# alessiodevoto/peekvit

Measured on AMD Instinct MI355X. Metric: images/sec ViT-B/16 fwd @ batch 2048, 224x224, higher is better.
Workload: dtype f16; 1 GPU; vit_b_16 forward, batch 2048/GPU, 224x224; global_batch=2048, parallelism=replicas x1 (batch-sharded, no collective), precision_mode=auto, streams=1, operands=IEEE fp16 operands, fp32 accumulate (same MFMA rate as bf16), range-guarded, range_guard_fallbacks=0

## Files before the change

### peekvit_amd/_build.py

```python
from __future__ import annotations

import glob
import os
import subprocess
import sys

HERE = os.path.dirname(os.path.abspath(__file__))
CSRC = os.path.join(HERE, "csrc")
LIB = os.path.join(HERE, "libpeekvit_hip.so")
LIB_F16 = os.path.join(HERE, "libpeekvit_hip_f16.so")
HIPCC = os.environ.get("HIPCC", "/opt/rocm/bin/hipcc")
FLAGS = ["--offload-arch=gfx950", "-O3", "-std=c++17", "-fPIC", "-Wno-unused-result"]
HEADERS = ("peekvit_hip.h", "peekvit_hip_moe.h", "peekvit_hip_ee.h", "peekvit_hip_sparse.h", "peekvit_hip_pct.h",
           "peekvit_hip_pct_train.h", "peekvit_hip_attn_stream.h", "peekvit_hip_pct_block.h", "peekvit_hip_rank_train.h", "peekvit_hip_rank_infer.h",
           "peekvit_hip_avit_train.h", "peekvit_hip_sparse_train.h", "peekvit_hip_avit_pack_train.h", "peekvit_hip_dropout.h", "peekvit_hip_sparse_long.h",
           "peekvit_hip_sparse_long_train.h", "peekvit_hip_avit_long.h")
FILE_FLAGS = {"pv_attention.hip": ["-mllvm", "-amdgpu-mfma-vgpr-form=1"], "pv_rowops.hip": ["-fno-slp-vectorize"],
              "pv_attention_stream.hip": ["-mllvm", "-amdgpu-mfma-vgpr-form=1"],
              "pv_ee.hip": ["-fno-slp-vectorize"],
              "pv_sparse.hip": ["-fno-slp-vectorize"],
              "pv_sparse_long.hip": ["-fno-slp-vectorize"],
              "pv_pct.hip": ["-fno-slp-vectorize"],
              "pv_pct_train.hip": ["-fno-slp-vectorize"],
              "pv_rank_train.hip": ["-fno-slp-vectorize"],
              "pv_avit_train.hip": ["-fno-slp-vectorize"],
              "pv_avit_pack_train.hip": ["-fno-slp-vectorize"],
              "pv_avit_long.hip": ["-fno-slp-vectorize"],
              "pv_dropout.hip": ["-fno-slp-vectorize"],
              "pv_sparse_train.hip": ["-fno-slp-vectorize", "-mllvm", "-amdgpu-mfma-vgpr-form=1"],
              "pv_sparse_long_train.hip": ["-fno-slp-vectorize"]}


def sources():
    return sorted(glob.glob(os.path.join(CSRC, "*.hip")))


def _stale() -> bool:
    if not os.path.exists(LIB) or not os.path.exists(LIB_F16):
        return True
    t = min(os.path.getmtime(LIB), os.path.getmtime(LIB_F16))
    deps = sources() + glob.glob(os.path.join(CSRC, "*.h")) + [os.path.join(os.path.dirname(HERE), "include", h) for h in HEADERS] + [os.path.abspath(__file__)]
    return any(os.path.getmtime(d) > t for d in deps)


def build(force: bool = False, verbose: bool = False) -> str:
    if not force and not _stale():
        return LIB
    procs = []
    variants = [("build", [], LIB), ("build_f16", ["-DPV_OPERAND_F16"], LIB_F16)]
    objs = {lib: [] for _, _, lib in variants}
    for sub, defs, lib in variants:
        objdir = os.path.join(HERE, sub)
        os.makedirs(objdir, exist_ok=True)
        for src in sources():
            obj = os.path.join(objdir, os.path.basename(src)[:-4] + ".o")
            objs[lib].append(obj)
            cmd = [HIPCC, *FLAGS, *FILE_FLAGS.get(os.path.basename(src), []), *defs, "-c", src, "-o", obj]
            if verbose:
                print(" ".join(cmd))
            procs.append((src, subprocess.Popen(cmd, stdout=subprocess.PIPE, stderr=subprocess.STDOUT)))
    for src, p in procs:
        out, _ = p.communicate()
        if p.returncode != 0:
            raise RuntimeError(f"hipcc failed on {src}:\n{out.decode(errors='replace')}")
    for _, _, lib in variants:
        cmd = [HIPCC, "--offload-arch=gfx950", "-shared", "-fPIC", "-o", lib, *objs[lib]]
        r = subprocess.run(cmd, stdout=subprocess.PIPE, stderr=subprocess.STDOUT)
        if r.returncode != 0:
            raise RuntimeError(f"link failed:\n{r.stdout.decode(errors='replace')}")
    return LIB


def build_variant(tag: str, defs, force: bool = False) -> str:
    lib = os.path.join(HERE, f"libpeekvit_hip_{tag}.so")
    deps = sources() + glob.glob(os.path.join(CSRC, "*.h")) + [os.path.join(os.path.dirname(HERE), "include", h) for h in HEADERS]
    if not force and os.path.exists(lib) and all(os.path.getmtime(d) <= os.path.getmtime(lib) for d in deps):
        return lib
    objdir = os.path.join(HERE, "build_" + tag)
    os.makedirs(objdir, exist_ok=True)
    procs, objs = [], []
    for src in sources():
        obj = os.path.join(objdir, os.path.basename(src)[:-4] + ".o")
        objs.append(obj)
        procs.append((src, subprocess.Popen([HIPCC, *FLAGS, *FILE_FLAGS.get(os.path.basename(src), []), *defs, "-c", src, "-o", obj],
                                            stdout=subprocess.PIPE, stderr=subprocess.STDOUT)))
    for src, p in procs:
        out, _ = p.communicate()
        if p.returncode != 0:
            raise RuntimeError(f"hipcc failed on {src}:\n{out.decode(errors='replace')}")
    r = subprocess.run([HIPCC, "--offload-arch=gfx950", "-shared", "-fPIC", "-o", lib, *objs], stdout=subprocess.PIPE, stderr=subprocess.STDOUT)
    if r.returncode != 0:
        raise RuntimeError(f"link failed:\n{r.stdout.decode(errors='replace')}")
    return lib


if __name__ == "__main__":
    print(build(force="--force" in sys.argv, verbose=True))
```

### peekvit_amd/_lib.py

```python
from __future__ import annotations

import ctypes as C
import os
import threading

import torch

from ._build import LIB

_i64, _f32, _p, _i32 = C.c_int64, C.c_float, C.c_void_p, C.c_int32

PV_EPI_BIAS_BF16, PV_EPI_BIAS_GELU_BF16, PV_EPI_BIAS_RES_F32, PV_EPI_BIAS_POS_F32 = 0, 1, 2, 3
PV_EPI_BIAS_F32, PV_EPI_BIAS_GELU_SPLIT_BF16 = 4, 5
PV_EPI_BIAS_GELU_PAIR_BF16, PV_EPI_GELU_GRAD_BF16 = 6, 7
PV_WS_TRANSPOSE_COLSUM, PV_WS_COLSUM, PV_WS_LAYERNORM_BWD, PV_WS_GEMM_COLSUM_PARTIAL, PV_WS_GEMM_SPLITK = 1, 2, 3, 4, 5


class GemmArgs(C.Structure):
    _fields_ = [("struct_size", C.c_uint64), ("A", _p), ("W", _p), ("bias", _p), ("out", _p), ("res", _p), ("row_scale", _p), ("pos", _p),
                ("M", _i64), ("N", _i64), ("K", _i64), ("lda", _i64), ("ldw", _i64), ("ldo", _i64), ("ldr", _i64),
                ("rows_per_img_in", _i64), ("rows_per_img_out", _i64), ("row_off", _i64), ("qcols", _i64),
                ("qscale", _f32), ("epilogue", _i32),
                ("ln_gamma", _p), ("ln_beta", _p), ("ln_row_scale", _p), ("ln_out", _p), ("ln_eps", _f32),
                ("ksplit", _i32), ("colsum_partial", _p),
# ... 86 lines not shown
    "pv_layernorm_f32_bf16": (C.c_int, [_p, _i64, _p, _p, _p, _p, _i64, _i64, _i64, _f32, _p]),
    "pv_mean_pool_f32": (C.c_int, [_p, _p, _i64, _i64, _i64, _p]),
    "pv_pct_head_f32": (C.c_int, [_p, _p, _p, _p, _p, _p, _p, _p, _i64, _i64, _i64, _i64, _p]),
}

SIGNATURES_PCT_TRAIN = {
    "pv_arpe_knn": (C.c_int, [_p, _p, _i64, _i64, _i64, _p]),
    "pv_arpe_pair_moments": (C.c_int, [_p, _p, _p, _p, _i64, _i64, _i64, _p]),
    "pv_arpe_pair_max": (C.c_int, [_p, _p, _p, _p, _p, _p, _p, _p, _i64, _i64, _i64, _p]),
    "pv_arpe_pair_bwd": (C.c_int, [_p, _p, _p, _p, _p, _p, _p, _i64, _i64, _p]),
}

SIGNATURES_ATTN_STREAM = {
    "pv_attention_stream_lse_bf16": (C.c_int, [_p, _p, _p, _i64, _i64, _i64, _i64, _p, _p]),
    "pv_attention_stream_bwd_bf16": (C.c_int, [_p, _p, _p, _p, _p, _p, _i64, _i64, _i64, _i64, _f32, _p]),
}

SIGNATURES_PCT_BLOCK = {
    "pv_layernorm_bwd_sum": (C.c_int, [_p, _p, _p, _p, _p, _p, _p, _p, _i64, _i64, _i64, _f32, C.c_int, _p]),
    "pv_attention_stream_bwd16_bf16": (C.c_int, [_p, _p, _p, _p, _p, _p, _p, _i64, _i64, _i64, _i64, _f32, _p]),
}

SIGNATURES_RANK_TRAIN = {
    "pv_rank_pack_f32": (C.c_int, [_p, _p, _p, _i64, _i64, _i64, _i64, _p]),
    "pv_rank_expand_f32": (C.c_int, [_p, _p, _i64, _i64, _i64, _i64, _p]),
    "pv_rank_reduce_f32": (C.c_int, [_p, _p, _i64, _i64, _i64, _i64, _p]),
    "pv_rank_unpack_grad_f32": (C.c_int, [_p, _p, _p, _i64, _i64, _i64, _i64, _p]),
    "pv_layernorm_f32_bf16_masked": (C.c_int, [_p, _p, _p, _p, _p, _p, _i64, _i64, _f32, _p]),
    "pv_layernorm_bwd_sum_masked": (C.c_int, [_p, _p, _p, _p, _p, _p, _p, _p, _p, _i64, _i64, _i64, _f32, C.c_int, _p]),
    "pv_attention_stream_lse_w_bf16": (C.c_int, [_p, _p, _p, _i64, _i64, _i64, _i64, _f32, _p, _p]),
    "pv_attention_stream_bwd16_w_bf16": (C.c_int, [_p, _p, _p, _p, _p, _p, _p, _i64, _i64, _i64, _i64, _f32, _f32, _p]),
}

SIGNATURES_RANK_INFER = {
    "pv_rank_order_gap": (C.c_int, [_p, _p, _p, _i64, _i64, _i64, _p]),
    "pv_layernorm_gather_f32_bf16": (C.c_int, [_p, _p, _p, _p, _p, _p, _i64, _i64, _i64, _i64, _f32, _p]),
}

SIGNATURES_AVIT_TRAIN = {
    "pv_avit_act_fwd": (C.c_int, [_p] * 16 + [_i64, _i64, _i64, _i64, _f32, _f32, _f32, C.c_int, _p]),
    "pv_avit_act_bwd": (C.c_int, [_p] * 9 + [_i64, _i64, _i64, _i64, _f32, C.c_int, _p]),
}

SIGNATURES_SPARSE_TRAIN = {
    "pv_attention_varlen_w_lse_bf16": (C.c_int, [_p, _p, _p, _p, _p, _i64, _i64, _i64, _i64, _p, _p]),
    "pv_attention_varlen_w_bwd16_bf16": (C.c_int, [_p, _p, _p, _p, _p, _p, _p, _p, _p, _i64, _i64, _i64, _i64, _f32, _p]),
    "pv_residual_pack_step_train": (C.c_int, [_p, _p, _p, _p, _i64, _i64, _i64, _p, _p, _p, _p, _f32, _f32, _p,
                                              _p, _p, _p, _p, _p, _p, _p, _p, _p, _p, _p, _f32, _p, _p, _p, _p]),
    "pv_residual_pack_step_bwd": (C.c_int, [_p] * 11 + [_i64, _i64, _i64, _p, _p, _f32, _p, _p, _p, _p, _p, _p]),
}

SIGNATURES_AVIT_PACK_TRAIN = {
    "pv_avit_pack_step_train": (C.c_int, [_p] * 4 + [_i64] * 4 + [_p] * 12 + [_i64, _p, _f32, _f32, _f32, C.c_int] + [_p] * 11),
    "pv_avit_pack_step_bwd": (C.c_int, [_p] * 16 + [_i64] * 6 + [_f32, C.c_int, _p]),
}

_u64 = C.c_uint64
SIGNATURES_DROPOUT = {
    "pv_dropout_keep_u8": (C.c_int, [_p, _u64, _u64, _i64, _i64, _f32, _p]),
    "pv_dropout_f32": (C.c_int, [_p, _p, _u64, _u64, _i64, _i64, _f32, _p]),
    "pv_dropout_residual": (C.c_int, [_p, _p, _p, _u64, _u64, _i64, _i64, _f32, _p]),
    "pv_dropout_bwd16": (C.c_int, [_p, _p, _u64, _u64, _i64, _i64, _f32, _p]),
    "pv_attention_stream_lse_drop_bf16": (C.c_int, [_p, _p, _p, _i64, _i64, _i64, _i64, _f32, _u64, _u64, _p, _p]),
    "pv_attention_stream_bwd16_drop_bf16": (C.c_int, [_p, _p, _p, _p, _p, _p, _p, _i64, _i64, _i64, _i64, _f32, _f32, _u64, _u64, _p]),
}

SIGNATURES_SPARSE_LONG = {
    "pv_attention_varlen_w_stream_bf16": SIGNATURES_SPARSE["pv_attention_varlen_w_bf16"],
    "pv_residual_pack_step_long": SIGNATURES_SPARSE["pv_residual_pack_step"],
}

SIGNATURES_SPARSE_LONG_TRAIN = {
    "pv_attention_varlen_w_stream_lse_bf16": SIGNATURES_SPARSE_TRAIN["pv_attention_varlen_w_lse_bf16"],
    "pv_attention_varlen_w_stream_bwd16_bf16": SIGNATURES_SPARSE_TRAIN["pv_attention_varlen_w_bwd16_bf16"],
    "pv_residual_pack_step_long_train": SIGNATURES_SPARSE_TRAIN["pv_residual_pack_step_train"],
    "pv_residual_pack_step_long_bwd": SIGNATURES_SPARSE_TRAIN["pv_residual_pack_step_bwd"],
}

SIGNATURES_AVIT_LONG = {
    "pv_avit_pack_step_long": SIGNATURES_AVIT_PACK_TRAIN["pv_avit_pack_step_train"],
    "pv_avit_pack_step_long_bwd": SIGNATURES_AVIT_PACK_TRAIN["pv_avit_pack_step_bwd"],
}

ABI_VERSION = 10
_lock = threading.Lock()
_libs: dict = {}

_OPERAND_DEFAULT = "bf16"
_tls = threading.local()
LIB_F16 = os.path.join(os.path.dirname(os.path.abspath(__file__)), "libpeekvit_hip_f16.so")


def current_operand() -> str:
    return getattr(_tls, "operand", _OPERAND_DEFAULT)


def set_operand(op: str) -> str:
    old = current_operand()
    _tls.operand = op
    return old


def __getattr__(name):
    if name == "OPERAND":
        return current_operand()
    raise AttributeError(f"module {__name__!r} has no attribute {name!r}")


def operand_dtype():
    import torch as _t
    return _t.float16 if current_operand() == "f16" else _t.bfloat16


class PeekvitHipError(RuntimeError):
    pass


def lib_path(operand: str = "bf16") -> str:
    return LIB_F16 if operand == "f16" else LIB


def load(operand=None):
    op = current_operand() if operand is None else operand
    lib = _libs.get(op)
    if lib is not None:
        return lib
    with _lock:
        lib = _libs.get(op)
        if lib is not None:
            return lib
        path = lib_path(op)
        if not os.path.exists(path):
            raise PeekvitHipError(
                f"{path} not found: the MI355X kernels are not built. Run `python -m peekvit_amd._build` "
                "(or __graft_entry__.build()); there is no fallback path.")
        lib = C.CDLL(path)
        for name, (res, args) in {**SIGNATURES, **SIGNATURES_MOE, **SIGNATURES_EE, **SIGNATURES_SPARSE, **SIGNATURES_PCT,
                                   **SIGNATURES_PCT_TRAIN, **SIGNATURES_ATTN_STREAM, **SIGNATURES_PCT_BLOCK, **SIGNATURES_RANK_TRAIN,
                                   **SIGNATURES_RANK_INFER, **SIGNATURES_AVIT_TRAIN, **SIGNATURES_SPARSE_TRAIN, **SIGNATURES_AVIT_PACK_TRAIN,
                                   **SIGNATURES_DROPOUT, **SIGNATURES_SPARSE_LONG, **SIGNATURES_SPARSE_LONG_TRAIN,
                                   **SIGNATURES_AVIT_LONG}.items():
            fn = getattr(lib, name)
            fn.restype, fn.argtypes = res, args
        if lib.pv_version() != ABI_VERSION:
            raise PeekvitHipError(f"{path} has ABI v{lib.pv_version()}, this package binds v{ABI_VERSION}: rebuild (python -m peekvit_amd._build)")
        if lib.pv_gemm_args_size() != C.sizeof(GemmArgs):
            raise PeekvitHipError(f"{path}: pv_gemm_args is {lib.pv_gemm_args_size()} bytes in the library, {C.sizeof(GemmArgs)} in this binding")
        if lib.pv_operand_type() != (1 if op == "f16" else 0):
            raise PeekvitHipError(f"{path} was built for a different operand type")
        _libs[op] = lib
    return lib


def check(code: int, what: str = "") -> None:
    if code != 0:
        msg = load().pv_error_string(code).decode()
        raise PeekvitHipError(f"{what}: {msg} (code {code})" if what else f"{msg} (code {code})")
```

### peekvit_amd/csrc/pv_gemm.hip

```cpp
#include "pv_rows.h"
#include "../../include/peekvit_hip_moe.h"
#include "pv_gelu_table.h"
#include <type_traits>
#include <cstdlib>

typedef __attribute__((ext_vector_type(8))) short s16x8;

#ifndef PV_STORE_NT
#define PV_STORE_NT 3
#endif
#define PV_STORE16(ptr, val) do { if (PV_STORE_NT & 1) __builtin_nontemporal_store((val), (ptr)); else *(ptr) = (val); } while (0)
#define PV_STORE32(ptr, val) do { if (PV_STORE_NT & 2) __builtin_nontemporal_store((val), (ptr)); else *(ptr) = (val); } while (0)
#ifndef PV_PF_MODE
#define PV_PF_MODE 2
#endif
#ifndef PV_EPI_PIPE
#define PV_EPI_PIPE 1
#endif

__device__ __forceinline__ float pv_fma_s(float a, float b, float c) {
    float r;
    asm("v_fma_f32 %0, %1, %2, %3" : "=v"(r) : "v"(a), "v"(b), "v"(c));
    return r;
}
__device__ __forceinline__ float pv_mul_s(float a, float b) {
    float r;
    asm("v_mul_f32 %0, %1, %2" : "=v"(r) : "v"(a), "v"(b));
    return r;
}
__device__ __forceinline__ float pv_gelu_poly(float x, const f32x4 c) {
    const pv_f32x2_t c02 = {c[0], c[1]}, c13 = {c[2], c[3]}, xx = {x, x};
    const pv_f32x2_t r = __builtin_elementwise_fma(c13, xx, c02);
    return pv_fma_s(x, pv_mul_s(x, r[1]), r[0]);
}
__device__ __forceinline__ void pv_gelu_bits2(float x0, float x1, uint32_t& b0, uint32_t& b1) {
    const pv_f32x2_t xs = {x0, x1}, sc = {PV_GELU_CUB_SCALE, PV_GELU_CUB_SCALE}, mg = {PV_GELU_CUB_MAGIC, PV_GELU_CUB_MAGIC};
    const pv_f32x2_t t = __builtin_elementwise_fma(xs, sc, mg);
    typedef __attribute__((ext_vector_type(2))) int pv_i32x2_t;
    const pv_i32x2_t ti = __builtin_bit_cast(pv_i32x2_t, t);
    const int lo = 0x4B400000, hi = 0x4B400000 + PV_GELU_CUB_N - 1;
    b0 = (uint32_t)min(max(ti[0], lo), hi);
    b1 = (uint32_t)min(max(ti[1], lo), hi);
}
#ifndef PV_GELU_GLOBAL_MODE
#define PV_GELU_GLOBAL_MODE 1
#endif
__device__ __forceinline__ float pv_gelu_poly_g(float x, f32x4 c) {
#if PV_GELU_GLOBAL_MODE == 0
    return pv_gelu_poly(x, c);
#elif PV_GELU_GLOBAL_MODE == 2
    asm volatile("s_nop 3" : "+v"(c));
    return pv_gelu_poly(x, c);
#elif PV_GELU_GLOBAL_MODE == 3
    pv_f32x2_t r;
    const pv_f32x2_t c02 = {c[0], c[1]}, c13 = {c[2], c[3]}, xx = {x, x};
    asm volatile("v_pk_fma_f32 %0, %1, %2, %3" : "=&v"(r) : "v"(c13), "v"(xx), "v"(c02));
    return pv_fma_s(x, pv_mul_s(x, r[1]), r[0]);
#elif PV_GELU_GLOBAL_MODE == 4
    const pv_f32x2_t c02 = {c[0], c[1]}, c13 = {c[2], c[3]}, xx = {x, x};
    const pv_f32x2_t r = __builtin_elementwise_fma(c13, xx, c02);
    return fmaf(x, x * r[1], r[0]);
#elif PV_GELU_GLOBAL_MODE == 6
    pv_f32x2_t r;
    const pv_f32x2_t c02 = {c[0], c[1]}, c13 = {c[2], c[3]}, xx = {x, 0.0f};
    asm volatile("v_pk_fma_f32 %0, %1, %2, %3 op_sel_hi:[1,0,1]" : "=&v"(r) : "v"(c13), "v"(xx), "v"(c02));
    return pv_fma_s(x, pv_mul_s(x, r[1]), r[0]);
#elif PV_GELU_GLOBAL_MODE == 9
    pv_f32x2_t r;
    const pv_f32x2_t c02 = {c[0], c[1]}, c13 = {c[2], c[3]}, xx = {0.0f, x};
    asm volatile("v_pk_fma_f32 %0, %1, %2, %3 op_sel:[0,1,0]" : "=&v"(r) : "v"(c13), "v"(xx), "v"(c02));
    return pv_fma_s(x, pv_mul_s(x, r[1]), r[0]);
#elif PV_GELU_GLOBAL_MODE == 7
    pv_f32x2_t c02 = {c[0], c[1]};
    const pv_f32x2_t c13 = {c[2], c[3]}, xx = {x, x};
    asm volatile("v_pk_fma_f32 %0, %1, %2, %0" : "+v"(c02) : "v"(c13), "v"(xx));
    return pv_fma_s(x, pv_mul_s(x, c02[1]), c02[0]);
#elif PV_GELU_GLOBAL_MODE == 8
    pv_f32x2_t c13 = {c[2], c[3]};
    const pv_f32x2_t c02 = {c[0], c[1]}, xx = {x, x};
    asm volatile("v_pk_fma_f32 %0, %0, %1, %2" : "+v"(c13) : "v"(xx), "v"(c02));
    return pv_fma_s(x, pv_mul_s(x, c13[1]), c13[0]);
#elif PV_GELU_GLOBAL_MODE == 5
    const float r0 = pv_fma_s(c[2], x, c[0]), r1 = pv_fma_s(c[3], x, c[1]);
    return pv_fma_s(x, pv_mul_s(x, r1), r0);
#else
    const float r0 = fmaf(c[2], x, c[0]), r1 = fmaf(c[3], x, c[1]);
    return pv_fma_s(x, pv_mul_s(x, r1), r0);
#endif
}
__device__ __forceinline__ void pv_gelu_lut2(float& x0, float& x1, const f32x4* tab) {
    uint32_t b0, b1;
    pv_gelu_bits2(x0, x1, b0, b1);
    const f32x4 c0 = tab[(b0 - 0x4B400000u) * PV_GELU_CUB_REP], c1 = tab[(b1 - 0x4B400000u) * PV_GELU_CUB_REP];
    x0 = pv_gelu_poly_g(x0, c0); x1 = pv_gelu_poly_g(x1, c1);
}
__device__ __forceinline__ void pv_gelu_lut2(float& x0, float& x1, const __attribute__((address_space(3))) f32x4* tab) {
    uint32_t b0, b1;
    pv_gelu_bits2(x0, x1, b0, b1);
    const uint32_t base = (uint32_t)(uintptr_t)tab - 0x40000000u;
    const f32x4 c0 = *(const __attribute__((address_space(3))) f32x4*)(uintptr_t)((b0 << 8) + base);
    const f32x4 c1 = *(const __attribute__((address_space(3))) f32x4*)(uintptr_t)((b1 << 8) + base);
    x0 = pv_gelu_poly(x0, c0); x1 = pv_gelu_poly(x1, c1);
}

__device__ __forceinline__ float pv_gelu_dpoly(float x, const f32x4 c) {
    const float t = pv_fma_s(pv_mul_s(c[3], 3.0f), x, pv_add_s(c[1], c[1]));
    return pv_fma_s(x, t, c[2]);
}
__device__ __forceinline__ void pv_gelu_dlut2(float& x0, float& x1, const f32x4* tab) {
    uint32_t b0, b1;
    pv_gelu_bits2(x0, x1, b0, b1);
    const f32x4 c0 = tab[(b0 - 0x4B400000u) * PV_GELU_CUB_REP], c1 = tab[(b1 - 0x4B400000u) * PV_GELU_CUB_REP];
    x0 = pv_gelu_dpoly(x0, c0); x1 = pv_gelu_dpoly(x1, c1);
}
__device__ __forceinline__ void pv_gelu_dlut2(float& x0, float& x1, const __attribute__((address_space(3))) f32x4* tab) {
    uint32_t b0, b1;
    pv_gelu_bits2(x0, x1, b0, b1);
    const uint32_t base = (uint32_t)(uintptr_t)tab - 0x40000000u;
    const f32x4 c0 = *(const __attribute__((address_space(3))) f32x4*)(uintptr_t)((b0 << 8) + base);
    const f32x4 c1 = *(const __attribute__((address_space(3))) f32x4*)(uintptr_t)((b1 << 8) + base);
    x0 = pv_gelu_dpoly(x0, c0); x1 = pv_gelu_dpoly(x1, c1);
}

struct GemmDev {
    const uint16_t* A;
    const uint16_t* W;
    const float* bias;
    void* out;
    const float* res;
    const float* row_scale;
    const float* pos;
    int M, N, K;
    int64_t lda, ldw, ldo, ldr;
    int rpi, rpo, row_off, qcols;
    float qscale;
    int tiles_m, tiles_n;
    int fr_full, fr_half;
    int fr_big;
    int gm;
    int gc;
    uint32_t* range_flag;
    float* rowsq_out;
    int res_scaled;
    int k_last;
    float* colsum_partial;
    uint16_t* x16_out;
    float* rowstat_out;
    const float* fold_stat;
    const float* fold_c1;
    const float* fold_c2;
    int ksplit;
    int k_slice;
    int64_t split_stride;
    const float* ln_gamma;
    const float* ln_beta;
    const float* ln_row_scale;
    uint16_t* ln_out;
    float ln_eps;
    const int* row_map;
    int map_rows;
#ifdef PV_STAMPS
    unsigned long long* dbg;
#endif
};

#ifdef PV_STAMPS
static unsigned long long* g_pv_dbg = nullptr;
extern "C" void pv_debug_set_stamp_buffer(void* p) { g_pv_dbg = (unsigned long long*)p; }
#define PV_STAMP(i)                                                                                  \
    do {                                                                                             \
        __builtin_amdgcn_sched_barrier(0);                                                           \
        unsigned long long t_;                                                                       \
        asm volatile("s_memtime %0\n\ts_waitcnt lgkmcnt(0)" : "=s"(t_)::"memory");                    \
        __builtin_amdgcn_sched_barrier(0);                                                           \
        if (threadIdx.x == 0 && p.dbg) p.dbg[pv_stamp_slot * 16 + (i)] = t_;                         \
    } while (0)
#else
#define PV_STAMP(i)
#endif

template <int AUX = 0>
__device__ __forceinline__ void pv_glds16(const void* gsrc, void* lds_wave_base) {
    __builtin_amdgcn_global_load_lds((const __attribute__((address_space(1))) void*)gsrc,
                                     (__attribute__((address_space(3))) void*)lds_wave_base, 16, 0, AUX);
}
#ifndef PV_GEMM_A_AUX
#define PV_GEMM_A_AUX 0
#endif
#ifndef PV_GEMM_W_AUX
#define PV_GEMM_W_AUX 0
#endif

__device__ __forceinline__ int pv_xcd_remap(int bid, int nwg) {
    const int q = nwg >> 3, r = nwg & 7, xcd = bid & 7, i = bid >> 3;
    return (xcd < r ? xcd * (q + 1) : r * (q + 1) + (xcd - r) * q) + i;
}

template <int EPI>
__device__ __forceinline__ f32x4 pv_epilogue_fetch(const GemmDev& p, int m, int n) {
    m = m < p.M ? m : p.M - 1;
    n = n + 4 <= p.N ? n : p.N - 4;
    if (EPI == PV_EPI_BIAS_RES_F32) {
        return *reinterpret_cast<const f32x4*>(p.res + (int64_t)m * p.ldr + n);
    } else if (EPI == PV_EPI_GELU_GRAD_BF16) {
        const u32x2 w = *reinterpret_cast<const u32x2*>(reinterpret_cast<const uint16_t*>(p.res) + (int64_t)m * p.ldr + n);
        return (f32x4){pv_unpack_lo(w[0]), pv_unpack_hi(w[0]), pv_unpack_lo(w[1]), pv_unpack_hi(w[1])};
    } else if (EPI == PV_EPI_BIAS_POS_F32) {
        const int img = m / p.rpi, pi = m - img * p.rpi;
        return *reinterpret_cast<const f32x4*>(p.pos + (int64_t)(p.row_off + pi) * p.N + n);
    }
    return (f32x4){0.f, 0.f, 0.f, 0.f};
}

template <int EPI, bool GUARD = true>
__device__ __forceinline__ void pv_epilogue_store(const GemmDev& p, int m, int n, f32x4 acc, f32x4 r, float row_scale, float& vmax) {
    if (GUARD && (m >= p.M || n >= p.N)) return;
    const float v0 = acc[0], v1 = acc[1], v2 = acc[2], v3 = acc[3];
    if (EPI == PV_EPI_BIAS_BF16) {
        const float s = n < p.qcols ? p.qscale : 1.0f;
        u32x2 o = {pv_pack_bf16x2_tracked(v0 * s, v1 * s, vmax), pv_pack_bf16x2_tracked(v2 * s, v3 * s, vmax)};
        *reinterpret_cast<u32x2*>(reinterpret_cast<uint16_t*>(p.out) + (int64_t)m * p.ldo + n) = o;
    } else if (EPI == PV_EPI_BIAS_GELU_BF16) {
        const f32x4* tab = reinterpret_cast<const f32x4*>(pv_gelu_cub) + (threadIdx.x & 15);
        float y0 = v0, y1 = v1, y2 = v2, y3 = v3;
        pv_gelu_lut2(y0, y1, tab); pv_gelu_lut2(y2, y3, tab);
        u32x2 o = {pv_pack_bf16x2_tracked(y0, y1, vmax), pv_pack_bf16x2_tracked(y2, y3, vmax)};
        *reinterpret_cast<u32x2*>(reinterpret_cast<uint16_t*>(p.out) + (int64_t)m * p.ldo + n) = o;
    } else if (EPI == PV_EPI_BIAS_RES_F32) {
        const float s = row_scale, t = p.res_scaled ? row_scale : 1.0f;
        float4 o = make_float4(fmaf(s, v0, t * r[0]), fmaf(s, v1, t * r[1]), fmaf(s, v2, t * r[2]), fmaf(s, v3, t * r[3]));
        *reinterpret_cast<float4*>(reinterpret_cast<float*>(p.out) + (int64_t)m * p.ldo + n) = o;
    } else if (EPI == PV_EPI_BIAS_F32) {
        const float s = n < p.qcols ? p.qscale : 1.0f;
        *reinterpret_cast<float4*>(reinterpret_cast<float*>(p.out) + (int64_t)m * p.ldo + n) = make_float4(v0 * s, v1 * s, v2 * s, v3 * s);
    } else if (EPI == PV_EPI_BIAS_GELU_SPLIT_BF16) {
        const f32x4* tab = reinterpret_cast<const f32x4*>(pv_gelu_cub) + (threadIdx.x & 15);
        float y0 = v0, y1 = v1, y2 = v2, y3 = v3;
        pv_gelu_lut2(y0, y1, tab); pv_gelu_lut2(y2, y3, tab);
        const PvHiLo a = pv_split2(y0, y1), b = pv_split2(y2, y3);
        uint16_t* o = reinterpret_cast<uint16_t*>(p.out) + (int64_t)m * p.ldo + n;
        *reinterpret_cast<u32x2*>(o) = (u32x2){a.hi, b.hi};
        *reinterpret_cast<u32x2*>(o + p.N) = (u32x2){a.lo, b.lo};
        *reinterpret_cast<u32x2*>(o + 2 * p.N) = (u32x2){a.hi, b.hi};
    } else if (EPI == PV_EPI_BIAS_GELU_PAIR_BF16) {
        const f32x4* tab = reinterpret_cast<const f32x4*>(pv_gelu_cub) + (threadIdx.x & 15);
        uint16_t* o = reinterpret_cast<uint16_t*>(p.out) + (int64_t)m * p.ldo + n;
        float y0 = v0, y1 = v1, y2 = v2, y3 = v3, d0 = v0, d1 = v1, d2 = v2, d3 = v3;
// ... 214 lines not shown
            bf16x8 xf[4], wf[4];
#pragma unroll
            for (int t = 0; t < 4; ++t) {
                xf[t] = *reinterpret_cast<const bf16x8*>(la + a_off + t * 2048 + fx);
                wf[t] = *reinterpret_cast<const bf16x8*>(lw + w_off + t * 2048 + fx);
            }
#pragma unroll
            for (int nt = 0; nt < 4; ++nt)
#pragma unroll
                for (int mt = 0; mt < 4; ++mt)
                    acc[nt][mt] = PV_MFMA_16x16x32(wf[nt], xf[mt], acc[nt][mt], 0, 0, 0);
        }
        if (kt + 1 < nk) put(cur ^ 1);
        asm volatile("s_waitcnt vmcnt(0)" ::: "memory");
        __syncthreads();
    }

    const int em = m0 + wm * 64 + (lane & 15);
    float dummy = 0.f;
    f32x4 rr[4][4];
#pragma unroll
    for (int mt = 0; mt < 4; ++mt)
#pragma unroll
        for (int nt = 0; nt < 4; ++nt) rr[mt][nt] = pv_epilogue_fetch<EPI>(p, em + mt * 16, en + nt * 16);
#pragma unroll
    for (int mt = 0; mt < 4; ++mt)
#pragma unroll
        for (int nt = 0; nt < 4; ++nt) asm volatile("" : "+v"(rr[mt][nt]));
    __builtin_amdgcn_sched_barrier(0);
    if (m0 + G1_BM <= p.M && n0 + G1_BN <= p.N) {
#pragma unroll
        for (int mt = 0; mt < 4; ++mt)
#pragma unroll
            for (int nt = 0; nt < 4; ++nt) pv_epilogue_store<EPI, false>(p, em + mt * 16, en + nt * 16, acc[nt][mt], rr[mt][nt], 1.0f, dummy);
    } else {
#pragma unroll
        for (int mt = 0; mt < 4; ++mt)
#pragma unroll
            for (int nt = 0; nt < 4; ++nt) pv_epilogue_store<EPI, true>(p, em + mt * 16, en + nt * 16, acc[nt][mt], rr[mt][nt], 1.0f, dummy);
    }
    pv_range_commit(vmax, p.range_flag);
}

extern "C" int pv_patch_embed_f32(const float* img, const uint16_t* W, const float* bias, const float* pos, float* tokens, int64_t B, int64_t C, int64_t R,
                                  int64_t P, int64_t D, int64_t S, int64_t row_off, uint32_t* range_flag, void* stream) {
    if (!img || !W || !pos || !tokens || B <= 0 || C <= 0 || R <= 0 || P <= 0 || D <= 0 || S <= 0 || row_off < 0) return PV_ERR_INVALID_ARG;
    if (R % P || P % 8 || (C * P * P) % G1_BK || D % 4 || R % 4 || ((uintptr_t)img & 15) || ((uintptr_t)W & 15) || ((uintptr_t)tokens & 15) || ((uintptr_t)pos & 15) ||
        (bias && ((uintptr_t)bias & 15)))
        return PV_ERR_UNSUPPORTED;
    const int64_t Wp = R / P, Np = Wp * Wp, M = B * Np;
    if (row_off + Np > S || M > 0x7fffffff || B * S > 0x7fffffff) return PV_ERR_INVALID_ARG;
    GemmDev p = {};
    p.W = W; p.bias = bias; p.out = tokens; p.pos = pos;
    p.M = (int)M; p.N = (int)D; p.K = (int)(C * P * P);
    p.ldw = p.K; p.ldo = D;
    p.rpi = (int)Np; p.rpo = (int)S; p.row_off = (int)row_off;
    p.qscale = 1.0f;
    p.tiles_m = (int)((M + G1_BM - 1) / G1_BM); p.tiles_n = (int)((D + G1_BN - 1) / G1_BN);
    p.range_flag = range_flag;
    const PatchGeom gm = {img, (int)C, (int)R, (int)P, (int)Wp, (int)Np};
    static PvPerDevice attr_set;
    const int lds = 2 * 2 * G1_TILE_BYTES;
    if (attr_set.first_use()) (void)hipFuncSetAttribute(reinterpret_cast<const void*>(pv_patch_embed_kernel), hipFuncAttributeMaxDynamicSharedMemorySize, lds);
    PV_LAUNCH(pv_patch_embed_kernel, dim3((unsigned)(p.tiles_m * p.tiles_n)), dim3(256), lds, (hipStream_t)stream, p, gm);
    return pv_check_launch();
}

template <int EPI>
static int pv_launch_gemm128(const GemmDev& p, hipStream_t stream) {
    static PvPerDevice attr_set;
    const int lds = 2 * 2 * G1_TILE_BYTES;
    if (attr_set.first_use()) {
        (void)hipFuncSetAttribute(reinterpret_cast<const void*>(pv_gemm128_kernel<EPI>), hipFuncAttributeMaxDynamicSharedMemorySize, lds);
    }
    PV_LAUNCH(pv_gemm128_kernel<EPI>, dim3((unsigned)(p.tiles_m * p.tiles_n * (p.ksplit > 1 ? p.ksplit : 1))), dim3(256), lds, stream, p);
    return pv_check_launch();
}

constexpr int G2_BM = 256, G2_BN = 256, G2_BK = 64;
constexpr int G2_HALF = 128 * G2_BK * 2;
constexpr int G2_BUF = 4 * G2_HALF;
constexpr int G2_LDS = 2 * G2_BUF;

template <int EPI, bool PF = false, bool FULL = false, bool PERM = false>
__device__ __forceinline__ void pv_gemm256_tile(const GemmDev& p, char* smem, const int m0, const int n0, const bool first = true,
                                                const bool has_next = false, const int nm0 = 0, const int nn0 = 0, const int wid_pf = 0, const int slot_pf = 0) {
    int tid_ = threadIdx.x;
    if (PF) {
        int l_;
        asm volatile("v_mbcnt_lo_u32_b32 %0, -1, 0\n\tv_mbcnt_hi_u32_b32 %0, -1, %0" : "=v"(l_));
        tid_ = wid_pf * 64 + l_;
    }
    int tid = tid_, lane = tid & 63;
    const int wid = PF ? wid_pf : __builtin_amdgcn_readfirstlane(tid >> 6);
    const int wr = wid >> 2, wc = wid & 3;
#ifdef PV_STAMPS
    const size_t pv_stamp_slot = PF ? (size_t)slot_pf : (size_t)blockIdx.x;
#endif
    constexpr int PFM = PV_PF_MODE;
    constexpr int PF_BIAS_BASE = G2_LDS + ((EPI == PV_EPI_BIAS_GELU_BF16 || EPI == PV_EPI_BIAS_GELU_SPLIT_BF16 || EPI == PV_EPI_BIAS_GELU_PAIR_BF16) ? PV_GELU_CUB_N * PV_GELU_CUB_REP * 16 : 0) + 4096;
    PV_STAMP(14);
#ifdef PV_STAMPS
    if (threadIdx.x == 0 && p.dbg) { unsigned long long rt_; asm volatile("s_memrealtime %0\n\ts_waitcnt lgkmcnt(0)" : "=s"(rt_)::"memory"); p.dbg[pv_stamp_slot * 16 + 13] = rt_; }
#endif

    const int srow = wid * 8 + (lane >> 3);
    const int schunk = (lane & 7) ^ ((lane >> 3) & 7);
    const char* const a_blk = reinterpret_cast<const char*>(p.A + (int64_t)m0 * p.lda);
    const char* const w_blk = reinterpret_cast<const char*>(p.W + (int64_t)n0 * p.ldw);
    uint32_t oa[2][2], ow[2][2];
#pragma unroll
    for (int h = 0; h < 2; ++h)
#pragma unroll
        for (int j = 0; j < 2; ++j) {
            int ra = h * 128 + j * 64 + srow; ra = (FULL || m0 + ra < p.M) ? ra : p.M - 1 - m0;
            const int q = j * 64 + srow;
            int rw = h * 128 + (q & ~31) + (((q & 15) >> 2) << 3) + (((q >> 4) & 1) << 2) + (q & 3);
            rw = (FULL || n0 + rw < p.N) ? rw : p.N - 1 - n0;
            oa[h][j] = (uint32_t)(ra * (int)p.lda + schunk * 8) * 2u;
            ow[h][j] = (uint32_t)(rw * (int)p.ldw + schunk * 8) * 2u;
        }
    char* const lds_piece = smem + wid * 1024;
    auto stage_a = [&](int buf, int h, int kt) {
        const char* src = a_blk + kt * (G2_BK * 2);
        pv_glds16<PV_GEMM_A_AUX>(src + oa[h][0], lds_piece + buf * G2_BUF + h * G2_HALF);
        pv_glds16<PV_GEMM_A_AUX>(src + oa[h][1], lds_piece + buf * G2_BUF + h * G2_HALF + 8192);
    };
    auto stage_b = [&](int buf, int h, int kt) {
        const char* src = w_blk + kt * (G2_BK * 2);
        pv_glds16<PV_GEMM_W_AUX>(src + ow[h][0], lds_piece + buf * G2_BUF + (2 + h) * G2_HALF);
        pv_glds16<PV_GEMM_W_AUX>(src + ow[h][1], lds_piece + buf * G2_BUF + (2 + h) * G2_HALF + 8192);
    };
    auto stage_next_piece = [&](int tm0, int tn0, int pc) __attribute__((always_inline)) {
        if (pc == 8) {
            if (p.bias && wid < 4) {
                const int c_ = tn0 + wid * 64 + lane < p.N ? tn0 + wid * 64 + lane : p.N - 1;
                __builtin_amdgcn_global_load_lds((const __attribute__((address_space(1))) void*)(p.bias + c_),
                                                 (__attribute__((address_space(3))) void*)(smem + PF_BIAS_BASE + wid * 256), 4, 0, 0);
            }
            return;
        }
        const int h = (pc >> 1) & 1, jj = pc & 1;
        const int sr = wid * 8 + (lane >> 3), sc = (lane & 7) ^ ((lane >> 3) & 7);
        if (pc < 4) {
            const char* const na = reinterpret_cast<const char*>(p.A + (int64_t)tm0 * p.lda);
            int ra = h * 128 + jj * 64 + sr; ra = tm0 + ra < p.M ? ra : p.M - 1 - tm0;
            pv_glds16<PV_GEMM_A_AUX>(na + (uint32_t)(ra * (int)p.lda + sc * 8) * 2u, lds_piece + h * G2_HALF + jj * 8192);
        } else {
            const char* const nw = reinterpret_cast<const char*>(p.W + (int64_t)tn0 * p.ldw);
            const int q = jj * 64 + sr;
            int rw = h * 128 + (q & ~31) + (((q & 15) >> 2) << 3) + (((q >> 4) & 1) << 2) + (q & 3);
            rw = tn0 + rw < p.N ? rw : p.N - 1 - tn0;
            pv_glds16<PV_GEMM_W_AUX>(nw + (uint32_t)(rw * (int)p.ldw + sc * 8) * 2u, lds_piece + (2 + h) * G2_HALF + jj * 8192);
        }
    };

    typedef __attribute__((address_space(3))) const char lds_cc;
    const int frow = (lane & 15) * 128;
    const int fx0 = ((lane >> 4) ^ (lane & 7)) << 4;
    lds_cc* const lds0 = (lds_cc*)smem;
    lds_cc* a_rd[2][2];
    lds_cc* b_rd[2][2];
#pragma unroll
    for (int b = 0; b < 2; ++b)
#pragma unroll
        for (int ks = 0; ks < 2; ++ks) {
            a_rd[b][ks] = lds0 + b * G2_BUF + wr * G2_HALF + frow + (fx0 ^ (ks << 6));
// ... 335 lines not shown
            if (pass == 1) {
                asm volatile("s_waitcnt lgkmcnt(0)" ::: "memory");
                __builtin_amdgcn_s_barrier();
            }
#pragma unroll
            for (int mt = 0; mt < 8; ++mt) {
                const int row = wr * 128 + mt * 16 + i16;
                float f_mean = 0.f, f_rstd = 1.f;
                if ((EPI == PV_EPI_BIAS_BF16 || EPI == PV_EPI_BIAS_GELU_BF16) && p.fold_stat) { f_mean = f_mean8[mt]; f_rstd = f_rstd8[mt]; }
#pragma unroll
                for (int u = 0; u < 2; ++u) {
                    f32x4 lo = acc[2 * u][mt], hi = acc[2 * u + 1][mt];
                    if ((EPI == PV_EPI_BIAS_BF16 || EPI == PV_EPI_BIAS_GELU_BF16) && p.fold_stat) {
#pragma unroll
                        for (int e = 0; e < 4; ++e) {
                            lo[e] = fmaf(f_rstd, fmaf(-f_mean, fc1[u][0][e], lo[e]), fc2[u][0][e]);
                            hi[e] = fmaf(f_rstd, fmaf(-f_mean, fc1[u][1][e], hi[e]), fc2[u][1][e]);
                        }
                    }
                    const float qs = (EPI == PV_EPI_BIAS_BF16 && en0 + u * 32 < p.qcols) ? p.qscale : 1.0f;
                    u32x4 pk;
                    if (PAIR) {
                        {
                            const __attribute__((address_space(3))) f32x4* tab = (const __attribute__((address_space(3))) f32x4*)(cimg + G2_LDS) + i16;
#pragma unroll
                            for (int e = 0; e < 4; e += 2) {
                                float t0 = lo[e], t1 = lo[e + 1], t2 = hi[e], t3 = hi[e + 1];
                                if (pass == 1) { pv_gelu_lut2(t0, t1, tab); pv_gelu_lut2(t2, t3, tab); }
                                else { pv_gelu_dlut2(t0, t1, tab); pv_gelu_dlut2(t2, t3, tab); }
                                lo[e] = t0; lo[e + 1] = t1; hi[e] = t2; hi[e + 1] = t3;
                            }
                        }
                        pk = (u32x4){pv_pack_bf16x2_tracked(lo[0], lo[1], vmax), pv_pack_bf16x2_tracked(lo[2], lo[3], vmax),
                                     pv_pack_bf16x2_tracked(hi[0], hi[1], vmax), pv_pack_bf16x2_tracked(hi[2], hi[3], vmax)};
                    } else if (EPI == PV_EPI_BIAS_GELU_BF16 || EPI == PV_EPI_BIAS_GELU_SPLIT_BF16) {
                        if (pass == 0) {
                            const __attribute__((address_space(3))) f32x4* tab = (const __attribute__((address_space(3))) f32x4*)(cimg + G2_LDS) + i16;
#pragma unroll
                            for (int e = 0; e < 4; e += 2) {
                                float t0 = lo[e], t1 = lo[e + 1], t2 = hi[e], t3 = hi[e + 1];
                                pv_gelu_lut2(t0, t1, tab); pv_gelu_lut2(t2, t3, tab);
                                lo[e] = t0; lo[e + 1] = t1; hi[e] = t2; hi[e + 1] = t3;
                            }
                            if (SPLIT) { acc[2 * u][mt] = lo; acc[2 * u + 1][mt] = hi; }
                        }
                        if (SPLIT) {
                            const PvHiLo s0 = pv_split2(lo[0], lo[1]), s1 = pv_split2(lo[2], lo[3]), s2 = pv_split2(hi[0], hi[1]), s3 = pv_split2(hi[2], hi[3]);
                            pk = pass == 0 ? (u32x4){s0.hi, s1.hi, s2.hi, s3.hi} : (u32x4){s0.lo, s1.lo, s2.lo, s3.lo};
                        } else {
                            pk = (u32x4){pv_pack_bf16x2_tracked(lo[0], lo[1], vmax), pv_pack_bf16x2_tracked(lo[2], lo[3], vmax),
                                         pv_pack_bf16x2_tracked(hi[0], hi[1], vmax), pv_pack_bf16x2_tracked(hi[2], hi[3], vmax)};
                        }
                    } else {
                        pk = (u32x4){pv_pack_bf16x2_tracked(lo[0] * qs, lo[1] * qs, vmax), pv_pack_bf16x2_tracked(lo[2] * qs, lo[3] * qs, vmax),
                                     pv_pack_bf16x2_tracked(hi[0] * qs, hi[1] * qs, vmax), pv_pack_bf16x2_tracked(hi[2] * qs, hi[3] * qs, vmax)};
                    }
                    const int c = wc * 8 + u * 4 + g;
                    *reinterpret_cast<__attribute__((address_space(3))) u32x4*>(cimg + row * 512 + ((c ^ (i16 & 7)) << 4)) = pk;
                }
            }
            asm volatile("s_waitcnt lgkmcnt(0)" ::: "memory");
            __builtin_amdgcn_s_barrier();
            uint16_t* const ob = reinterpret_cast<uint16_t*>(p.out) + n0 + (lane & 31) * 8;
#pragma unroll
            for (int j = 0; j < 16; ++j) {
                const int row = wid * 32 + 2 * j + (lane >> 5);
                const u32x4 v = *reinterpret_cast<const __attribute__((address_space(3))) u32x4*>(cimg + row * 512 + (((lane & 31) ^ (row & 7)) << 4));
                if (m0 + row < p.M && n0 + (lane & 31) * 8 < p.N) {
                    uint16_t* o = ob + (int64_t)(m0 + row) * p.ldo;
                    if (PAIR) {
                        *reinterpret_cast<u32x4*>(pass == 0 ? o + p.N : o) = v;
                    } else if (!SPLIT) {
                        *reinterpret_cast<u32x4*>(o) = v;
                    } else if (pass == 0) {
                        *reinterpret_cast<u32x4*>(o) = v;
                        *reinterpret_cast<u32x4*>(o + 2 * p.N) = v;
                    } else {
                        *reinterpret_cast<u32x4*>(o + p.N) = v;
                    }
                }
            }
        }
        if (!SPLIT) pv_range_commit(vmax, p.range_flag);
    } else {
        constexpr bool DG = EPI == PV_EPI_GELU_GRAD_BF16;
        float cs8[DG ? 8 : 1];
        if constexpr (DG) {
#pragma unroll
            for (int e = 0; e < 8; ++e) cs8[e] = 0.f;
        }
        u32x4 dg[DG ? 2 : 1][DG ? 4 : 1];
        const int dg_col = n0 + 8 * (lane & 31);
        const bool dg_col_ok = FULL || dg_col + 8 <= p.N;
        float vmax = 0.f;
        lds_c* const img = cimg + G2_BUF;
        const bool col_ok = FULL || n0 + lane * 4 < p.N;
        const int ncol = col_ok ? n0 + lane * 4 : 0;
        f32x4 rr[2][8];
        float rsc[2] = {1.0f, 1.0f};
        auto row_of = [&](int q, int j) -> int64_t {
            int m = m0 + q * 64 + wid * 8 + j;
            m = (FULL || m < p.M) ? m : p.M - 1;
            if (PERM) return p.row_map[m];
            if (EPI == PV_EPI_BIAS_POS_F32) { const int img_ = m / p.rpi, pi = m - img_ * p.rpi; return (int64_t)img_ * p.rpo + p.row_off + pi; }
            return m;
        };
        auto fetch = [&](int q) __attribute__((always_inline)) {
            if constexpr (DG) {
#pragma unroll
                for (int jj = 0; jj < 4; ++jj) {
                    int m = m0 + q * 64 + wid * 8 + 2 * jj + (lane >> 5);
                    m = (FULL || m < p.M) ? m : p.M - 1;
                    dg[q & 1][jj] = *reinterpret_cast<const u32x4*>(reinterpret_cast<const uint16_t*>(p.res) + (int64_t)m * p.ldr + (dg_col_ok ? dg_col : 0));
                }
                return;
            }
#pragma unroll
            for (int j = 0; j < 8; ++j) {
                int m = m0 + q * 64 + wid * 8 + j;
                m = (FULL || m < p.M) ? m : p.M - 1;
                f32x4& r = rr[q & 1][j];
                if (EPI == PV_EPI_BIAS_F32) {
                    r = (f32x4){0.f, 0.f, 0.f, 0.f};
                } else if (EPI == PV_EPI_BIAS_RES_F32) {
                    int64_t rm = m;
                    if (PERM) { const int s_ = p.row_map[m]; rm = (s_ >= 0 && s_ < p.map_rows) ? s_ : 0; }
                    r = *reinterpret_cast<const f32x4*>(p.res + rm * p.ldr + ncol);
                } else {
                    const int img_ = m / p.rpi, pi = m - img_ * p.rpi;
                    r = *reinterpret_cast<const f32x4*>(p.pos + (int64_t)(p.row_off + pi) * p.N + ncol);
                }
            }
            if (EPI == PV_EPI_BIAS_RES_F32 && p.row_scale) {
                int m = m0 + q * 64 + wid * 8 + (lane & 7);
                rsc[q & 1] = p.row_scale[m < p.M ? m : p.M - 1];
            }
        };
        fetch(0);
        fetch(1);
        if (PFM == 2 && pf_next) {
#pragma unroll
            for (int pc = 0; pc < 9; ++pc) stage_next_piece(nm0, nn0, pc);
        }
#pragma unroll
        for (int q = 0; q < 4; ++q) {
            if (q > 0) __builtin_amdgcn_s_barrier();
            if (wr == (q >> 1)) {
#pragma unroll
                for (int ml = 0; ml < 4; ++ml) {
                    const int mt = 4 * (q & 1) + ml, row = ml * 16 + i16;
#pragma unroll
                    for (int nt = 0; nt < 4; ++nt) {
                        const int c = wc * 16 + (nt >> 1) * 8 + g * 2 + (nt & 1);
                        *reinterpret_cast<__attribute__((address_space(3))) f32x4*>(img + row * 1024 + ((c ^ (i16 & 7)) << 4)) = acc[nt][mt];
                    }
                }
            }
            asm volatile("s_waitcnt lgkmcnt(0)" ::: "memory");
            __builtin_amdgcn_s_barrier();
            if (PFM == 1 && q == 0 && pf_next) asm volatile("s_waitcnt vmcnt(0)" ::: "memory");
            float fs[8], fq[8];
            if constexpr (DG) {
#pragma unroll
                for (int jj = 0; jj < 4; ++jj) {
                    const int row = wid * 8 + 2 * jj + (lane >> 5), c0 = 2 * (lane & 31);
                    const f32x4 va = *reinterpret_cast<const __attribute__((address_space(3))) f32x4*>(img + row * 1024 + ((c0 ^ (row & 7)) << 4));
// ... 2 lines not shown
                    const u32x4 pk = {pv_pack_bf16x2(pv_mul_s(va[0], pv_unpack_lo(d[0])), pv_mul_s(va[1], pv_unpack_hi(d[0]))),
                                      pv_pack_bf16x2(pv_mul_s(va[2], pv_unpack_lo(d[1])), pv_mul_s(va[3], pv_unpack_hi(d[1]))),
                                      pv_pack_bf16x2(pv_mul_s(vb[0], pv_unpack_lo(d[2])), pv_mul_s(vb[1], pv_unpack_hi(d[2]))),
                                      pv_pack_bf16x2(pv_mul_s(vb[2], pv_unpack_lo(d[3])), pv_mul_s(vb[3], pv_unpack_hi(d[3])))};
                    const int mrow = m0 + q * 64 + row;
                    if (FULL || (mrow < p.M && dg_col_ok)) {
                        PV_STORE16(reinterpret_cast<u32x4*>(reinterpret_cast<uint16_t*>(p.out) + (int64_t)mrow * p.ldo + dg_col), pk);
#pragma unroll
                        for (int e = 0; e < 4; ++e) {
                            cs8[2 * e] = pv_add_s(cs8[2 * e], pv_unpack_lo(pk[e]));
                            cs8[2 * e + 1] = pv_add_s(cs8[2 * e + 1], pv_unpack_hi(pk[e]));
                        }
                    }
                }
            } else
#pragma unroll
            for (int j = 0; j < 8; ++j) {
                const int row = wid * 8 + j;
                const int64_t orow = row_of(q, j);
                const f32x4 v = *reinterpret_cast<const __attribute__((address_space(3))) f32x4*>(img + row * 1024 + ((lane ^ (row & 7)) << 4));
                const f32x4 r = rr[q & 1][j];
                const float sc = (EPI == PV_EPI_BIAS_RES_F32 && p.row_scale)
                                     ? __builtin_bit_cast(float, __builtin_amdgcn_readlane(__builtin_bit_cast(int, rsc[q & 1]), j)) : 1.0f;
                f32x4 o;
                if (EPI == PV_EPI_BIAS_F32) {
                    const float qs = ncol < p.qcols ? p.qscale : 1.0f;
                    o = (f32x4){v[0] * qs, v[1] * qs, v[2] * qs, v[3] * qs};
                } else if (EPI == PV_EPI_BIAS_RES_F32) {
                    const float tr = p.res_scaled ? sc : 1.0f;
                    o = (f32x4){fmaf(sc, v[0], tr * r[0]), fmaf(sc, v[1], tr * r[1]), fmaf(sc, v[2], tr * r[2]), fmaf(sc, v[3], tr * r[3])};
                }
                else o = (f32x4){r[0] + v[0], r[1] + v[1], r[2] + v[2], r[3] + v[3]};
                const bool ok = (FULL || (m0 + q * 64 + row < p.M && col_ok)) && (!PERM || (orow >= 0 && orow < p.map_rows));
                if (ok) PV_STORE32(reinterpret_cast<f32x4*>(reinterpret_cast<float*>(p.out) + orow * p.ldo + ncol), o);
                if (EPI == PV_EPI_BIAS_RES_F32 && p.rowsq_out)
                    fq[j] = ok ? pv_add_s(pv_add_s(o[0] * o[0], o[1] * o[1]), pv_add_s(o[2] * o[2], o[3] * o[3])) : 0.f;
                if (EPI == PV_EPI_BIAS_RES_F32 && p.x16_out) {
                    if (ok)
                        PV_STORE16(reinterpret_cast<u32x2*>(p.x16_out + orow * (int64_t)p.N + ncol), ((u32x2){pv_pack_bf16x2_tracked(o[0], o[1], vmax), pv_pack_bf16x2_tracked(o[2], o[3], vmax)}));
                    fs[j] = ok ? pv_add_s(pv_add_s(o[0], o[1]), pv_add_s(o[2], o[3])) : 0.f;
                    fq[j] = ok ? pv_add_s(pv_add_s(o[0] * o[0], o[1] * o[1]), pv_add_s(o[2] * o[2], o[3] * o[3])) : 0.f;
                }
            }
            if (q + 2 < 4) fetch(q + 2);
            {
                const int r_ = (lane >> 3) & 7, mrow = m0 + q * 64 + wid * 8 + r_;
                if (EPI == PV_EPI_BIAS_RES_F32 && p.rowsq_out && !p.x16_out) {
                    const float tq = pv_reduce8_rows(fq, lane);
                    if ((lane & 7) == 0 && mrow < p.M) p.rowsq_out[(int64_t)(n0 / G2_BN) * p.M + mrow] = tq;
                }
                if (EPI == PV_EPI_BIAS_RES_F32 && p.x16_out) {
                    const float ts = pv_reduce8_rows(fs, lane), tq = pv_reduce8_rows(fq, lane);
                    if ((lane & 7) == 0 && mrow < p.M)
                        *reinterpret_cast<float2*>(p.rowstat_out + ((int64_t)(n0 / G2_BN) * p.M + mrow) * 2) = make_float2(ts, tq);
                }
            }
        }
        if (EPI == PV_EPI_BIAS_RES_F32 && p.x16_out) pv_range_commit(vmax, p.range_flag);
        if (EPI == PV_EPI_GELU_GRAD_BF16 && p.colsum_partial) {
            asm volatile("s_waitcnt lgkmcnt(0)" ::: "memory");
            __builtin_amdgcn_s_barrier();
            if constexpr (DG) {
#pragma unroll
                for (int e = 0; e < 8; ++e) cs8[e] = pv_add_s(cs8[e], __shfl_xor(cs8[e], 32, 64));
                if (lane < 32) {
                    *reinterpret_cast<__attribute__((address_space(3))) f32x4*>(cimg + G2_BUF + wid * 1024 + lane * 32) = (f32x4){cs8[0], cs8[1], cs8[2], cs8[3]};
                    *reinterpret_cast<__attribute__((address_space(3))) f32x4*>(cimg + G2_BUF + wid * 1024 + lane * 32 + 16) = (f32x4){cs8[4], cs8[5], cs8[6], cs8[7]};
                }
            }
            asm volatile("s_waitcnt lgkmcnt(0)" ::: "memory");
            __builtin_amdgcn_s_barrier();
            if (tid < 256 && n0 + tid < p.N) {
                float t = 0.f;
#pragma unroll
                for (int w = 0; w < 8; ++w) t += *reinterpret_cast<const __attribute__((address_space(3))) float*>(cimg + G2_BUF + w * 1024 + tid * 4);
                p.colsum_partial[(int64_t)(m0 / G2_BM) * p.N + n0 + tid] = t;
            }
        }
    }
    if (PFM == 2 && pf_next) {
        const bool full = FULL || (m0 + G2_BM <= p.M && n0 + G2_BN <= p.N);
        constexpr bool B16 = EPI == PV_EPI_BIAS_BF16 || EPI == PV_EPI_BIAS_GELU_BF16 || EPI == PV_EPI_BIAS_GELU_PAIR_BF16 || EPI == PV_EPI_GELU_GRAD_BF16;
        if (!full) asm volatile("s_waitcnt vmcnt(0)" ::: "memory");
        else if (B16) asm volatile("s_waitcnt vmcnt(16)" ::: "memory");
        else asm volatile("s_waitcnt vmcnt(32)" ::: "memory");
    }
    PV_STAMP(3);
#ifdef PV_STAMPS
    if (threadIdx.x == 0 && p.dbg) {
        unsigned hw, xcc;
        asm volatile("s_getreg_b32 %0, hwreg(HW_REG_HW_ID)" : "=s"(hw));
        asm volatile("s_getreg_b32 %0, hwreg(HW_REG_XCC_ID)" : "=s"(xcc));
        p.dbg[pv_stamp_slot * 16 + 5] = ((unsigned long long)(xcc & 0xf) << 32) | hw;
    }
    asm volatile("s_waitcnt vmcnt(0)" ::: "memory");
    PV_STAMP(4);
    if (threadIdx.x == 0 && p.dbg) { unsigned long long rt_; asm volatile("s_memrealtime %0\n\ts_waitcnt lgkmcnt(0)" : "=s"(rt_)::"memory"); p.dbg[pv_stamp_slot * 16 + 7] = rt_; }
#endif
}

template <int EPI>
__global__ __launch_bounds__(512) void pv_gemm256_kernel(const GemmDev p_in) {
    extern __shared__ __attribute__((aligned(16))) char smem[];
    GemmDev p = p_in;
    const int ntiles = p.tiles_m * p.tiles_n;
    const int slice = blockIdx.x / ntiles;
    if (p.ksplit > 1) {
        p.A += (int64_t)slice * p.k_slice; p.W += (int64_t)slice * p.k_slice; p.K = p.k_slice;
        p.out = reinterpret_cast<float*>(p.out) + slice * p.split_stride;
        if (slice) p.bias = nullptr;
    }
    const int tile = pv_xcd_remap(blockIdx.x - slice * ntiles, ntiles);
    const int nfull = p.tiles_n / p.gc;
    const int ch = min(tile / (p.gc * p.tiles_m), nfull);
    const int r = tile - ch * p.gc * p.tiles_m;
    const int cw = ch < nfull ? p.gc : p.tiles_n - nfull * p.gc;
    const int grp = r / (p.gm * cw), rem = r - grp * (p.gm * cw);
    const int gsz = min(p.gm, p.tiles_m - grp * p.gm);
    const int tnl = rem / gsz, tm = grp * p.gm + (rem - tnl * gsz);
    const int m0 = tm * G2_BM, n0 = (ch * p.gc + tnl) * G2_BN;
    if (m0 + G2_BM <= p.M && n0 + G2_BN <= p.N) pv_gemm256_tile<EPI, false, true>(p, smem, m0, n0);
    else pv_gemm256_tile<EPI, false, false>(p, smem, m0, n0);
}

template <int EPI>
__global__ __launch_bounds__(512) void pv_gemm256_pf_kernel(const GemmDev p) {
    extern __shared__ __attribute__((aligned(16))) char smem[];
    const int ntiles = p.tiles_m * p.tiles_n;
    const int xcd = blockIdx.x & 7, j = blockIdx.x >> 3, per = gridDim.x >> 3;
    const int q8 = ntiles >> 3, r8 = ntiles & 7;
    const int start = xcd < r8 ? xcd * (q8 + 1) : r8 * (q8 + 1) + (xcd - r8) * q8;
    const int cnt = q8 + (xcd < r8 ? 1 : 0);
    const int nfull = p.tiles_n / p.gc;
    auto decode = [&](int tile, int& m0, int& n0) {
        const int ch = min(tile / (p.gc * p.tiles_m), nfull);
        const int r = tile - ch * p.gc * p.tiles_m;
        const int cw = ch < nfull ? p.gc : p.tiles_n - nfull * p.gc;
        const int grp = r / (p.gm * cw), rem = r - grp * (p.gm * cw);
        const int gsz = min(p.gm, p.tiles_m - grp * p.gm);
        const int tnl = rem / gsz, tm = grp * p.gm + (rem - tnl * gsz);
        m0 = tm * G2_BM; n0 = (ch * p.gc + tnl) * G2_BN;
    };
    const int wid = __builtin_amdgcn_readfirstlane((int)threadIdx.x >> 6);
    int m0 = 0, n0 = 0, nm0 = 0, nn0 = 0;
    if (j < cnt) decode(start + j, m0, n0);
    for (int i = j; i < cnt; i += per) {
        const bool has_next = i + per < cnt;
        if (has_next) decode(start + i + per, nm0, nn0);
        if (m0 + G2_BM <= p.M && n0 + G2_BN <= p.N) pv_gemm256_tile<EPI, true, true>(p, smem, m0, n0, i == j, has_next, nm0, nn0, wid, start + i);
        else pv_gemm256_tile<EPI, true, false>(p, smem, m0, n0, i == j, has_next, nm0, nn0, wid, start + i);
        asm volatile("s_waitcnt lgkmcnt(0)" ::: "memory");
        __builtin_amdgcn_s_barrier();
        __builtin_amdgcn_sched_barrier(0);
        m0 = nm0; n0 = nn0;
    }
}

struct PvGroupDev {
    const int* tile_expert;
    int64_t w_stride;
    int E;
};

template <int EPI>
__global__ __launch_bounds__(512) void pv_gemm256_kernel(const GemmDev p_in, const PvGroupDev g) {
    extern __shared__ __attribute__((aligned(16))) char smem[];
    const int ntiles = p_in.tiles_m * p_in.tiles_n;
    const int tile = pv_xcd_remap(blockIdx.x, ntiles);
    const int tm = tile / p_in.tiles_n, tn = tile - tm * p_in.tiles_n;
    const int e = __builtin_amdgcn_readfirstlane(g.tile_expert[tm]);
    if (e < 0 || e >= g.E) return;
    GemmDev p = p_in;
    p.W += (int64_t)e * g.w_stride;
    if (p.bias) p.bias += (int64_t)e * p.N;
    const int m0 = tm * G2_BM, n0 = tn * G2_BN;
    constexpr bool PERM = EPI == PV_EPI_BIAS_RES_F32;
    if (n0 + G2_BN <= p.N) pv_gemm256_tile<EPI, false, true, PERM>(p, smem, m0, n0);
    else pv_gemm256_tile<EPI, false, false, PERM>(p, smem, m0, n0);
}

__global__ __launch_bounds__(512) void pv_gemm256_tn_kernel(const GemmDev p_in) {
    extern __shared__ __attribute__((aligned(16))) char smem[];
    GemmDev p = p_in;
    const int ntiles = p.tiles_m * p.tiles_n;
    int slice, tile;
    if (p.gm != 0) {
        const int l = pv_xcd_remap(blockIdx.x, ntiles * p.ksplit);
        slice = l / ntiles; tile = l - slice * ntiles;
    } else {
        slice = blockIdx.x / ntiles; tile = pv_xcd_remap(blockIdx.x - slice * ntiles, ntiles);
    }
    p.A += (int64_t)slice * p.k_slice * p.lda; p.W += (int64_t)slice * p.k_slice * p.ldw;
    p.K = slice == p.ksplit - 1 ? p.k_last : p.k_slice;
    p.out = reinterpret_cast<float*>(p.out) + slice * p.split_stride;
    const int tm = tile / p.tiles_n, tn = tile - tm * p.tiles_n;
    const int m0 = tm * G2_BM, n0 = tn * G2_BN;

    const int tid = threadIdx.x, lane = tid & 63;
    const int wid = __builtin_amdgcn_readfirstlane(tid >> 6);
    const int wr = wid >> 2, wc = wid & 3;
    constexpr int SLOT = 2 * G2_HALF;

    const int sw_s = ((lane >> 4) << 2) | ((wid & 1) << 1);
    const int scol = ((lane & 15) ^ sw_s) * 8;
    const char* const a_blk = reinterpret_cast<const char*>(p.A + m0);
    const char* const w_blk = reinterpret_cast<const char*>(p.W + n0);
    const uint32_t oa = (uint32_t)((4 * wid + (lane >> 4)) * (int)p.lda + scol) * 2u;
    const uint32_t ow = (uint32_t)((4 * wid + (lane >> 4)) * (int)p.ldw + scol) * 2u;
    const int a_h1 = m0 + 256 <= p.M ? 256 : 0, w_h1 = n0 + 256 <= p.N ? 256 : 0;
    char* const lds_piece = smem + wid * 1024;
    const int64_t a_step = (int64_t)G2_BK * p.lda * 2, w_step = (int64_t)G2_BK * p.ldw * 2;
    auto stage_a = [&](int buf, int h, int kt) __attribute__((always_inline)) {
        const char* src = a_blk + kt * a_step + (h ? a_h1 : 0);
        pv_glds16(src + oa, lds_piece + h * SLOT + buf * G2_HALF);
        pv_glds16(src + (a_step >> 1) + oa, lds_piece + h * SLOT + buf * G2_HALF + 8192);
    };
    auto stage_b = [&](int buf, int h, int kt) __attribute__((always_inline)) {
        const char* src = w_blk + kt * w_step + (h ? w_h1 : 0);
        pv_glds16(src + ow, lds_piece + (2 + h) * SLOT + buf * G2_HALF);
        pv_glds16(src + (w_step >> 1) + ow, lds_piece + (2 + h) * SLOT + buf * G2_HALF + 8192);
    };

    typedef __attribute__((address_space(3))) const char lds_cc;
    const int g = lane >> 4, i16 = lane & 15, tq = i16 >> 2, tp = i16 & 3;
    const int rl = 4 * g + tq;
    const int sw_l = (tq << 2) | ((g & 1) << 1);
    lds_cc* const lds0 = (lds_cc*)smem;
    lds_cc* a_rd[8];
    lds_cc* b_rd[4];
#pragma unroll
    for (int t = 0; t < 8; ++t) {
        a_rd[t] = lds0 + wr * SLOT + rl * 256 + (((2 * t + (tp >> 1)) ^ sw_l) << 4) + ((tp & 1) << 3);
        asm volatile("" : "+v"(a_rd[t]));
    }
#pragma unroll
    for (int t = 0; t < 4; ++t) {
        b_rd[t] = lds0 + (2 + (wc >> 1)) * SLOT + rl * 256 + (((2 * ((wc & 1) * 4 + t) + (tp >> 1)) ^ sw_l) << 4) + ((tp & 1) << 3);
        asm volatile("" : "+v"(b_rd[t]));
// ... 179 lines not shown
#pragma unroll
            for (int j = 0; j < NCH; ++j) r.v[j] = make_float4(raw[rb][j][0], raw[rb][j][1], raw[rb][j][2], raw[rb][j][3]);
            pv_ln_row<NCH>(r, p.ln_gamma, p.ln_beta, D, nvec, lane, p.ln_eps);
            const float sc = p.ln_row_scale ? p.ln_row_scale[m] : 1.0f;
            u32x2* o = reinterpret_cast<u32x2*>(p.ln_out + (int64_t)m * D);
#pragma unroll
            for (int j = 0; j < NCH; ++j) {
                const int idx = lane + 64 * j;
                if (idx < nvec) {
                    u32x2 pk = {pv_pack_bf16x2(r.v[j].x * sc, r.v[j].y * sc), pv_pack_bf16x2(r.v[j].z * sc, r.v[j].w * sc)};
                    o[idx] = pk;
                }
            }
        }
    }
}

template <int EPI>
__global__ __launch_bounds__(512) void pv_gemm256_rows_kernel(const GemmDev p) {
    extern __shared__ __attribute__((aligned(16))) char smem[];
    const int m0 = pv_xcd_remap(blockIdx.x, p.tiles_m) * G2_BM;
    for (int tn = 0; tn < p.tiles_n; ++tn) {
        pv_gemm256_tile<EPI>(p, smem, m0, tn * G2_BN);
        asm volatile("s_waitcnt lgkmcnt(0)" ::: "memory");
        __builtin_amdgcn_s_barrier();
    }
    asm volatile("s_waitcnt vmcnt(0)" ::: "memory");
    __builtin_amdgcn_s_barrier();
    const int nch = (p.N / 4 + 63) / 64;
    if (nch <= 1) pv_fused_ln_rows<1>(p, m0);
    else if (nch == 2) pv_fused_ln_rows<2>(p, m0);
    else if (nch == 3) pv_fused_ln_rows<3>(p, m0);
    else if (nch == 4) pv_fused_ln_rows<4>(p, m0);
    else if (nch <= 8) pv_fused_ln_rows<8>(p, m0);
    else pv_fused_ln_rows<16>(p, m0);
}

#ifndef PV_GEMM_PF_DEFAULT
#define PV_GEMM_PF_DEFAULT 1
#endif
static int g_pv_pf = -1;
extern "C" void pv_debug_set_gemm_pf(int on) { g_pv_pf = on; }
static bool pv_gemm_pf_enabled() {
    static const int env = [] { const char* e = getenv("PV_GEMM_PF"); return e ? atoi(e) : PV_GEMM_PF_DEFAULT; }();
    return g_pv_pf >= 0 ? g_pv_pf != 0 : env != 0;
}
static int pv_cu_count() {
    static int cached[64] = {};
    int d = 0;
    if (hipGetDevice(&d) != hipSuccess || d < 0 || d >= 64) return 0;
    if (cached[d] == 0) {
        int n = 0;
        if (hipDeviceGetAttribute(&n, hipDeviceAttributeMultiprocessorCount, d) != hipSuccess) n = 0;
        cached[d] = n > 0 ? n : -1;
    }
    return cached[d] > 0 ? cached[d] : 0;
}

template <int EPI>
static int pv_launch_gemm256(const GemmDev& p, hipStream_t stream) {
    static PvPerDevice attr_set;
    constexpr int lds = G2_LDS + ((EPI == PV_EPI_BIAS_GELU_BF16 || EPI == PV_EPI_BIAS_GELU_SPLIT_BF16 || EPI == PV_EPI_BIAS_GELU_PAIR_BF16)
                                        ? PV_GELU_CUB_N * PV_GELU_CUB_REP * 16 : 0)
                        + ((EPI == PV_EPI_BIAS_BF16 || EPI == PV_EPI_BIAS_GELU_BF16) ? 4096 : 0);
    constexpr int lds_pf = EPI == PV_EPI_GELU_GRAD_BF16 ? lds
                         : G2_LDS + ((EPI == PV_EPI_BIAS_GELU_BF16 || EPI == PV_EPI_BIAS_GELU_SPLIT_BF16 || EPI == PV_EPI_BIAS_GELU_PAIR_BF16) ? PV_GELU_CUB_N * PV_GELU_CUB_REP * 16 : 0) + 4096 + 1024;
    constexpr bool PF_OK = EPI != PV_EPI_BIAS_GELU_SPLIT_BF16 && (PV_EPI_PIPE || (EPI != PV_EPI_BIAS_BF16 && EPI != PV_EPI_BIAS_GELU_BF16 && EPI != PV_EPI_BIAS_GELU_PAIR_BF16));
    if (attr_set.first_use()) {
        (void)hipFuncSetAttribute(reinterpret_cast<const void*>(static_cast<void (*)(const GemmDev)>(pv_gemm256_kernel<EPI>)), hipFuncAttributeMaxDynamicSharedMemorySize, lds);
        if (PF_OK) (void)hipFuncSetAttribute(reinterpret_cast<const void*>(pv_gemm256_pf_kernel<EPI>), hipFuncAttributeMaxDynamicSharedMemorySize, lds_pf);
    }
    if (PF_OK) {
        const int cus = pv_cu_count();
        if (pv_gemm_pf_enabled() && p.ksplit <= 1 && p.K >= 4 * G2_BK && (int64_t)p.tiles_m * p.tiles_n >= 2 * (int64_t)cus && cus >= 8 &&
            !(EPI == PV_EPI_GELU_GRAD_BF16 && p.bias)) {
            PV_LAUNCH(pv_gemm256_pf_kernel<EPI>, dim3((unsigned)(cus & ~7)), dim3(512), lds_pf, stream, p);
            return pv_check_launch();
        }
    }
    PV_LAUNCH((static_cast<void (*)(const GemmDev)>(pv_gemm256_kernel<EPI>)), dim3((unsigned)(p.tiles_m * p.tiles_n * (p.ksplit > 1 ? p.ksplit : 1))), dim3(512), lds, stream, p);
    return pv_check_launch();
}

template <int EPI>
static int pv_launch_gemm256_rows(const GemmDev& p, hipStream_t stream) {
    static PvPerDevice attr_set;
    if (attr_set.first_use()) {
        (void)hipFuncSetAttribute(reinterpret_cast<const void*>(pv_gemm256_rows_kernel<EPI>), hipFuncAttributeMaxDynamicSharedMemorySize, G2_LDS);
    }
    PV_LAUNCH(pv_gemm256_rows_kernel<EPI>, dim3((unsigned)p.tiles_m), dim3(512), G2_LDS, stream, p);
    return pv_check_launch();
}

template <int N_>
__device__ __forceinline__ void pv_wait_vmcnt() { asm volatile("s_waitcnt vmcnt(%0)" ::"n"(N_) : "memory"); }

struct PvFrCounts { int pro; int v[3][4]; };
constexpr PvFrCounts pv_fr_counts(int NPH, int PW, int AP = 2) {
    constexpr int NK = 8;
    int kind[512] = {}, tile[512] = {};
    int n = 0;
    auto issue = [&](int k, int t, int cnt) { for (int i = 0; i < cnt; ++i) { kind[n] = k; tile[n] = t; ++n; } };
    auto younger = [&](int k, int t) { int last = -1; for (int i = 0; i < n; ++i) if (kind[i] == k && tile[i] == t) last = i; return n - 1 - last; };
    PvFrCounts c = {};
    issue(0, 0, AP);
    for (int g = 0; g < NPH; ++g) issue(1 + g, 0, PW);
    issue(0, 1, AP);
    for (int g = 0; g < NPH - 1; ++g) issue(1 + g, 1, PW);
    c.pro = younger(1, 0);
    for (int s = 0; s < NK; ++s)
        for (int j = 0; j < NPH; ++j) {
            if (j == 0) { if (s + 1 < NK) issue(NPH, s + 1, PW); }
            else if (s + 2 < NK) { if (j == 1) { issue(0, s + 2, AP); issue(1, s + 2, PW); } else issue(j, s + 2, PW); }
            int w = 0;
            if (j < NPH - 1) w = younger(2 + j, s);
            else if (s + 1 < NK) w = younger(1, s + 1);
            const int mode = s == NK - 1 ? 2 : s == NK - 2 ? 1 : 0;
            if (mode != 0 || s == 3) c.v[mode][j] = w;
        }
    return c;
}

template <int NT, int DPH, int MT>
__device__ __forceinline__ void pv_fullrow_body(const GemmDev& p, char* const smem, const int m0, const bool half) {
    constexpr bool DP = DPH > 0;
    static_assert(MT == 4 || (MT == 5 && DP && NT <= 6), "160-row tiles: deep-pipelined loop, N <= 384");
    constexpr int N = 64 * NT, BM = 32 * MT, BK = 64;
    constexpr int AP = (BM + 63) / 64;
    constexpr int A_BYTES = AP * 64 * BK * 2;
    constexpr int BUF = A_BYTES + N * BK * 2;
    const int tid = threadIdx.x, lane = tid & 63;
    const int wid = __builtin_amdgcn_readfirstlane(tid >> 6);
    const int wm = wid >> 2, wn = wid & 3;
#ifdef PV_STAMPS
    const size_t pv_stamp_slot = (size_t)blockIdx.x;
    if (threadIdx.x == 0 && p.dbg) { unsigned long long rt_; asm volatile("s_memrealtime %0\n\ts_waitcnt lgkmcnt(0)" : "=s"(rt_)::"memory"); p.dbg[pv_stamp_slot * 16 + 5] = rt_; p.dbg[pv_stamp_slot * 16 + 7] = (unsigned long long)(half ? 1 : MT == 5 ? 2 : 0); }
#endif
    PV_STAMP(0);
    const bool skip_mm = half && wm == 1;
    const int g = lane >> 4, i16 = lane & 15;

    constexpr bool BIAS_LDS = DP && NT <= 6;
    constexpr int BIAS_OFF = 2 * BUF;
    f32x4 acc[NT][MT];
    if constexpr (BIAS_LDS) {
        if (p.bias && wid < NT)
            __builtin_amdgcn_global_load_lds((const __attribute__((address_space(1))) void*)(p.bias + wid * 64 + lane),
                                             (__attribute__((address_space(3))) void*)(smem + BIAS_OFF + wid * 256), 4, 0, 0);
    } else {
#pragma unroll
        for (int nt = 0; nt < NT; ++nt) {
            f32x4 b4 = {0.f, 0.f, 0.f, 0.f};
            if (p.bias) b4 = *reinterpret_cast<const f32x4*>(p.bias + wn * 16 * NT + nt * 16 + 4 * g);
#pragma unroll
            for (int mt = 0; mt < MT; ++mt) acc[nt][mt] = b4;
        }
#pragma unroll
        for (int nt = 0; nt < NT; ++nt)
#pragma unroll
            for (int mt = 0; mt < MT; ++mt) asm volatile("" : "+v"(acc[nt][mt]));
        __builtin_amdgcn_sched_barrier(0);
    }

    constexpr int KC = NT;
    const int q4 = lane >> 4, l16 = lane & 15;
    constexpr int RB = (NT <= 6) ? 2 : 1;
// ... 289 lines not shown
        const int nb8 = (p.fr_big + 7) >> 3;
        const int x = blockIdx.x & 7, j = blockIdx.x >> 3;
        if (j < nb8) {
            const int q = p.fr_big >> 3, r = p.fr_big & 7;
            if (j >= q + (x < r ? 1 : 0)) return;
            m0_ = p.fr_full * BM + ((x < r ? x * (q + 1) : r * (q + 1) + (x - r) * q) + j) * 160;
            big = true;
        } else m0_ = (x * (p.fr_full >> 3) + (j - nb8)) * BM;
    } else if (p.fr_full > 0) {
        const int x = blockIdx.x & 7, j = blockIdx.x >> 3, fper = p.fr_full >> 3, q = p.fr_half >> 3, r = p.fr_half & 7;
        if (j < fper) m0_ = (x * fper + j) * BM;
        else {
            const int hj = j - fper;
            if (hj >= q + (x < r ? 1 : 0)) return;
            m0_ = p.fr_full * BM + ((x < r ? x * (q + 1) : r * (q + 1) + (x - r) * q) + hj) * 64;
            half = true;
        }
    } else m0_ = pv_xcd_remap(blockIdx.x, p.tiles_m) * BM;
    if constexpr (DPH > 0 && NT <= 6) {
        if (big) { pv_fullrow_body<NT, DPH, 5>(p, smem, m0_, false); return; }
    }
    pv_fullrow_body<NT, DPH, 4>(p, smem, m0_, half);
}

static int g_pv_frdp = -1;
extern "C" void pv_debug_set_fullrow_dp(int on) { g_pv_frdp = on; }
static int pv_fullrow_dp_mode() {
    static const int env = [] { const char* e = getenv("PV_FULLROW_DP"); return e ? atoi(e) : 1; }();
    return g_pv_frdp >= 0 ? g_pv_frdp : env;
}
static int g_pv_frsplit = -1;
extern "C" void pv_debug_set_fullrow_split(int on) { g_pv_frsplit = on; }
static int pv_fullrow_split_mode() {
    static const int env = [] { const char* e = getenv("PV_FULLROW_SPLIT"); return e ? atoi(e) : 2; }();
    return g_pv_frsplit >= 0 ? g_pv_frsplit : env;
}
static bool pv_fullrow_split_enabled() { return pv_fullrow_split_mode() != 0; }

template <int NT>
static int pv_launch_gemm_fullrow(const GemmDev& p, hipStream_t stream) {
    static PvPerDevice attr_set;
    constexpr int lds = 2 * (128 * 64 * 2 + 64 * NT * 64 * 2);
    constexpr int lds_big = 2 * (192 * 64 * 2 + 64 * NT * 64 * 2) + 256 * NT;
    if (attr_set.first_use()) {
        (void)hipFuncSetAttribute(reinterpret_cast<const void*>(pv_gemm_fullrow_kernel<NT, 0>), hipFuncAttributeMaxDynamicSharedMemorySize, lds);
        (void)hipFuncSetAttribute(reinterpret_cast<const void*>(pv_gemm_fullrow_kernel<NT, 2>), hipFuncAttributeMaxDynamicSharedMemorySize, NT <= 6 ? lds_big : lds);
    }
    GemmDev q = p;
    q.fr_full = 0; q.fr_half = 0; q.fr_big = 0;
    unsigned grid = (unsigned)p.tiles_m;
    const int cus = pv_cu_count() & ~7;
    const bool dp = p.K % 128 == 0 && pv_fullrow_dp_mode() != 0;
    if (pv_fullrow_split_mode() == 2 && NT <= 6 && dp && cus >= 8 && p.tiles_m > cus) {
        const int rounds = p.tiles_m / cus;
        const int64_t rem = p.M - (int64_t)rounds * cus * 128;
        if (rem > 0 && rem <= (int64_t)cus * 32) {
            q.fr_full = (rounds - 1) * cus;
            q.fr_big = (int)((p.M - (int64_t)q.fr_full * 128 + 159) / 160);
            grid = 8u * (unsigned)((q.fr_big + 7) / 8) + (unsigned)q.fr_full;
        }
    }
    if (pv_fullrow_split_mode() == 3 && NT <= 6 && dp && cus >= 8 && p.tiles_m > cus) {
        q.fr_full = 0; q.fr_big = (int)((p.M + 159) / 160);
        grid = 8u * (unsigned)((q.fr_big + 7) / 8);
    }
    if (q.fr_big == 0 && pv_fullrow_split_enabled() && cus >= 8 && p.tiles_m > cus) {
        const int full = p.tiles_m / cus * cus;
        const int64_t rem = p.M - (int64_t)full * 128;
        if (rem > 0 && rem <= (int64_t)cus * 64) {
            q.fr_full = full; q.fr_half = (int)((rem + 63) / 64);
            grid = 8u * (unsigned)(full / 8 + (q.fr_half + 7) / 8);
        }
    }
    if (dp) PV_LAUNCH((pv_gemm_fullrow_kernel<NT, 2>), dim3(grid), dim3(512), q.fr_big > 0 ? lds_big : NT <= 6 ? lds + 256 * NT : lds, stream, q);
    else PV_LAUNCH((pv_gemm_fullrow_kernel<NT, 0>), dim3(grid), dim3(512), lds, stream, q);
    return pv_check_launch();
}

static int g_pv_raster_gm = 0, g_pv_raster_gc = 0;
extern "C" void pv_debug_set_gemm_raster(int gm, int gc) { g_pv_raster_gm = gm; g_pv_raster_gc = gc; }
static int g_pv_fullrow = -1;
extern "C" void pv_debug_set_gemm_fullrow(int on) { g_pv_fullrow = on; }

static int pv_gemm_dispatch(const pv_gemm_args* a, void* stream, bool query_only);
extern "C" int pv_gemm_bf16(const pv_gemm_args* a, void* stream) { return pv_gemm_dispatch(a, stream, false); }
extern "C" int pv_gemm_tile_rows(const pv_gemm_args* a) {
    if (!a || a->struct_size != sizeof(pv_gemm_args)) return PV_ERR_INVALID_ARG;
    pv_gemm_args q = *a;
    q.colsum_partial = nullptr; q.x16_out = nullptr; q.rowstat_out = nullptr; q.fold_stat = nullptr; q.rowsq_out = nullptr;
    return pv_gemm_dispatch(&q, nullptr, true);
}
static int pv_gemm_dispatch(const pv_gemm_args* a, void* stream, bool query_only) {
    if (!a || a->struct_size != sizeof(pv_gemm_args)) return PV_ERR_INVALID_ARG;
    if (!a->A || !a->W || !a->out || a->M <= 0 || a->N <= 0 || a->K <= 0) return PV_ERR_INVALID_ARG;
    if (a->K % 64 || a->N % 4) return PV_ERR_UNSUPPORTED;
    if (a->lda % 8 || a->ldw % 8 || a->ldo % 4 || a->lda < a->K || a->ldw < a->K || a->ldo < a->N) return PV_ERR_INVALID_ARG;
    if (((uintptr_t)a->A & 15) || ((uintptr_t)a->W & 15) || ((uintptr_t)a->out & 15) || (a->bias && ((uintptr_t)a->bias & 15))) return PV_ERR_INVALID_ARG;
    if (a->M > 0x7fffffff || a->N > 0x7fffffff || a->K > 0x7fffffff) return PV_ERR_UNSUPPORTED;
    if ((uintptr_t)a->range_flag & 3) return PV_ERR_INVALID_ARG;
    GemmDev p;
    p.range_flag = a->range_flag;
    p.rowsq_out = a->rowsq_out;
    if (a->rowsq_out && (a->epilogue != PV_EPI_BIAS_RES_F32 || ((uintptr_t)a->rowsq_out & 3) || a->ln_out || a->x16_out)) return PV_ERR_INVALID_ARG;
    p.A = a->A; p.W = a->W; p.bias = a->bias; p.out = a->out; p.res = a->res; p.row_scale = a->row_scale; p.pos = a->pos;
    p.res_scaled = a->res_scaled;
    if (a->res_scaled && (a->epilogue != PV_EPI_BIAS_RES_F32 || !a->row_scale)) return PV_ERR_INVALID_ARG;
    p.M = (int)a->M; p.N = (int)a->N; p.K = (int)a->K;
    p.lda = a->lda; p.ldw = a->ldw; p.ldo = a->ldo; p.ldr = a->ldr;
    p.rpi = (int)a->rows_per_img_in; p.rpo = (int)a->rows_per_img_out; p.row_off = (int)a->row_off;
    p.qcols = (int)a->qcols; p.qscale = a->qscale;
#ifdef PV_STAMPS
    p.dbg = g_pv_dbg;
#endif
    p.colsum_partial = a->colsum_partial;
    p.x16_out = a->x16_out; p.rowstat_out = a->rowstat_out; p.fold_stat = a->fold_stat; p.fold_c1 = a->fold_c1; p.fold_c2 = a->fold_c2;
    if ((a->x16_out != nullptr) != (a->rowstat_out != nullptr)) return PV_ERR_INVALID_ARG;
    if (a->x16_out && (a->epilogue != PV_EPI_BIAS_RES_F32 || ((uintptr_t)a->x16_out & 7) || ((uintptr_t)a->rowstat_out & 7))) return PV_ERR_INVALID_ARG;
    if (a->fold_stat && ((a->epilogue != PV_EPI_BIAS_BF16 && a->epilogue != PV_EPI_BIAS_GELU_BF16) || a->bias || !a->fold_c1 || !a->fold_c2 || a->N < 8 ||
                         ((uintptr_t)a->fold_stat & 7) || ((uintptr_t)a->fold_c1 & 15) || ((uintptr_t)a->fold_c2 & 15))) return PV_ERR_INVALID_ARG;
    if (a->colsum_partial && (a->epilogue != PV_EPI_GELU_GRAD_BF16 || ((uintptr_t)a->colsum_partial & 15))) return PV_ERR_INVALID_ARG;
    p.ksplit = a->ksplit > 1 ? a->ksplit : 1; p.k_slice = (int)(a->K / p.ksplit); p.split_stride = a->M * a->ldo;
    if (p.ksplit > 1) {
        if (a->epilogue != PV_EPI_BIAS_F32 || a->qcols != 0 || a->ln_out || a->K % (p.ksplit * 64)) return PV_ERR_INVALID_ARG;
    }
    p.ln_gamma = a->ln_gamma; p.ln_beta = a->ln_beta; p.ln_row_scale = a->ln_row_scale; p.ln_out = a->ln_out; p.ln_eps = a->ln_eps;
    hipStream_t s = (hipStream_t)stream;
    if (a->ln_out) {
        if (a->epilogue != PV_EPI_BIAS_RES_F32 || !a->ln_gamma || !a->ln_beta) return PV_ERR_INVALID_ARG;
        if (!(a->N == 256 || a->N == 384 || a->N == 512) && (a->N % G2_BN || a->N > 4096 || a->K % (2 * G2_BK))) return PV_ERR_UNSUPPORTED;
        if (a->ldo != a->N) return PV_ERR_UNSUPPORTED;
        if (((uintptr_t)a->ln_out & 7) || ((uintptr_t)a->ln_gamma & 15) || ((uintptr_t)a->ln_beta & 15)) return PV_ERR_INVALID_ARG;
    }
    if (a->epilogue == PV_EPI_BIAS_RES_F32 && (!a->res || a->ldr % 4 || a->ldr < a->N || ((uintptr_t)a->res & 15))) return PV_ERR_INVALID_ARG;
    if (a->epilogue == PV_EPI_GELU_GRAD_BF16 && (!a->res || a->ldr % 4 || a->ldr < a->N || ((uintptr_t)a->res & 7))) return PV_ERR_INVALID_ARG;
    if (a->epilogue == PV_EPI_BIAS_POS_F32 &&
        (!a->pos || a->rows_per_img_in <= 0 || a->rows_per_img_out < a->rows_per_img_in + a->row_off || a->row_off < 0 || ((uintptr_t)a->pos & 15)))
        return PV_ERR_INVALID_ARG;
    static const int force = [] { const char* e = getenv("PV_GEMM_TILE"); return e ? atoi(e) : 0; }();
    const int tn256 = (p.N + G2_BN - 1) / G2_BN;
    const bool n_ok = p.N % 128 == 0 && (int64_t)tn256 * G2_BN * 3 <= (int64_t)p.N * 4;
    const int k_eff = p.ksplit > 1 ? p.k_slice : p.K;
    const int64_t tiles256 = (int64_t)((p.M + G2_BM - 1) / G2_BM) * tn256;
    const bool ragged_short = (int64_t)tn256 * G2_BN * 3 >= (int64_t)p.N * 4 && k_eff <= 512;
    const bool feat = a->colsum_partial || a->x16_out || a->fold_stat || a->rowsq_out;
    const bool pipe16 = a->epilogue == PV_EPI_BIAS_BF16 || a->epilogue == PV_EPI_BIAS_GELU_BF16 || a->epilogue == PV_EPI_BIAS_GELU_PAIR_BF16;
    const bool ld_ok256 = a->lda <= (0x7fffffffLL - 56) / 255 && a->ldw <= (0x7fffffffLL - 56) / 255 &&
                          (!pipe16 || a->ldo <= (0x7fffffffLL - 248 - (a->epilogue == PV_EPI_BIAS_GELU_PAIR_BF16 ? a->N : 0)) / 255);
    const bool big = ld_ok256 && !((a->epilogue == PV_EPI_BIAS_BF16 || a->epilogue == PV_EPI_BIAS_F32) && p.qcols % 8) &&
                     (force == 256 || (force != 128 && n_ok && k_eff % (2 * G2_BK) == 0 &&
                                       ((tiles256 >= 128 && !ragged_short) || feat ||
                                        (p.ksplit > 1 && (int64_t)p.M * p.N >= 256 * 256 && tiles256 * p.ksplit >= 64))));
    if (big && a->epilogue == PV_EPI_GELU_GRAD_BF16 && (p.N % 8 || a->ldr % 8 || a->ldo % 8 || ((uintptr_t)a->res & 15) || ((uintptr_t)a->out & 15))) return PV_ERR_UNSUPPORTED;
    if (big && (k_eff % (2 * G2_BK) || k_eff < 2 * G2_BK)) return PV_ERR_UNSUPPORTED;
    if ((a->colsum_partial || a->x16_out || a->fold_stat || a->rowsq_out) && !big) return PV_ERR_UNSUPPORTED;
    static const int fullrow_env = [] { const char* e = getenv("PV_GEMM_FULLROW"); return e ? atoi(e) : 1; }();
    const bool fullrow_shape = a->epilogue == PV_EPI_BIAS_RES_F32 && (p.N == 256 || p.N == 384 || p.N == 512) && p.ksplit <= 1 && !feat &&
                               (g_pv_fullrow >= 0 ? g_pv_fullrow != 0 : fullrow_env != 0) && force == 0;
    if (a->ln_out && !fullrow_shape && !ld_ok256) return PV_ERR_UNSUPPORTED;
    if (query_only) return big ? G2_BM : G1_BM;
    if ((a->epilogue == PV_EPI_BIAS_BF16 || a->epilogue == PV_EPI_BIAS_F32) && p.qcols % 4) return PV_ERR_UNSUPPORTED;
    static const int gm_env = [] { const char* e = getenv("PV_GEMM_GM"); return e ? atoi(e) : 0; }();
    const int bm = big ? G2_BM : G1_BM, bn = big ? G2_BN : G1_BN;
    p.tiles_m = (p.M + bm - 1) / bm; p.tiles_n = (p.N + bn - 1) / bn;
    p.gm = p.tiles_n >= 8 ? (p.tiles_n >= 12 ? 6 : 8) : (p.tiles_n >= 6 ? 4 : 1);
    p.gc = p.tiles_n >= 12 ? 6 : p.tiles_n;
    if (gm_env > 0) p.gm = gm_env;
    if (g_pv_raster_gm > 0) p.gm = g_pv_raster_gm;
    if (g_pv_raster_gc > 0) p.gc = g_pv_raster_gc < p.tiles_n ? g_pv_raster_gc : p.tiles_n;
    if ((int64_t)p.tiles_m * p.tiles_n > 0x7fffffff) return PV_ERR_UNSUPPORTED;
    if (a->res_scaled && (fullrow_shape || a->ln_out)) return PV_ERR_UNSUPPORTED;
    if (fullrow_shape && (a->ln_out || (p.M + 127) / 128 >= 96)) {
        p.tiles_m = (p.M + 127) / 128; p.tiles_n = 1;
        return p.N == 256 ? pv_launch_gemm_fullrow<4>(p, s) : p.N == 384 ? pv_launch_gemm_fullrow<6>(p, s) : pv_launch_gemm_fullrow<8>(p, s);
    }
    if (a->ln_out) {
        p.gm = 1; p.gc = p.tiles_n;
        p.tiles_m = (p.M + G2_BM - 1) / G2_BM; p.tiles_n = p.N / G2_BN;
        return pv_launch_gemm256_rows<PV_EPI_BIAS_RES_F32>(p, s);
    }
    switch (a->epilogue) {
        case PV_EPI_BIAS_BF16: return big ? pv_launch_gemm256<PV_EPI_BIAS_BF16>(p, s) : pv_launch_gemm128<PV_EPI_BIAS_BF16>(p, s);
        case PV_EPI_BIAS_GELU_BF16: return big ? pv_launch_gemm256<PV_EPI_BIAS_GELU_BF16>(p, s) : pv_launch_gemm128<PV_EPI_BIAS_GELU_BF16>(p, s);
        case PV_EPI_BIAS_RES_F32: return big ? pv_launch_gemm256<PV_EPI_BIAS_RES_F32>(p, s) : pv_launch_gemm128<PV_EPI_BIAS_RES_F32>(p, s);
        case PV_EPI_BIAS_POS_F32: return big ? pv_launch_gemm256<PV_EPI_BIAS_POS_F32>(p, s) : pv_launch_gemm128<PV_EPI_BIAS_POS_F32>(p, s);
        case PV_EPI_BIAS_F32: return big ? pv_launch_gemm256<PV_EPI_BIAS_F32>(p, s) : pv_launch_gemm128<PV_EPI_BIAS_F32>(p, s);
        case PV_EPI_BIAS_GELU_SPLIT_BF16:
            if (a->ldo < 3 * a->N) return PV_ERR_INVALID_ARG;
            return big ? pv_launch_gemm256<PV_EPI_BIAS_GELU_SPLIT_BF16>(p, s) : pv_launch_gemm128<PV_EPI_BIAS_GELU_SPLIT_BF16>(p, s);
        case PV_EPI_BIAS_GELU_PAIR_BF16:
            if (a->ldo < 2 * a->N) return PV_ERR_INVALID_ARG;
            return big ? pv_launch_gemm256<PV_EPI_BIAS_GELU_PAIR_BF16>(p, s) : pv_launch_gemm128<PV_EPI_BIAS_GELU_PAIR_BF16>(p, s);
        case PV_EPI_GELU_GRAD_BF16: return big ? pv_launch_gemm256<PV_EPI_GELU_GRAD_BF16>(p, s) : pv_launch_gemm128<PV_EPI_GELU_GRAD_BF16>(p, s);
        default: return PV_ERR_INVALID_ARG;
    }
}

extern "C" int pv_gemm_grouped_bf16(const pv_gemm_args* a, const int32_t* tile_expert, int64_t tiles_m, int64_t E, int64_t w_stride,
                                    const int32_t* perm, int64_t out_rows, void* stream) {
    if (!a || a->struct_size != sizeof(pv_gemm_args)) return PV_ERR_INVALID_ARG;
    if (!a->A || !a->W || !a->out || !tile_expert || a->M <= 0 || a->N <= 0 || a->K <= 0 || tiles_m <= 0) return PV_ERR_INVALID_ARG;
    if (E < 1 || E > PV_MOE_MAX_EXPERTS || a->M != tiles_m * G2_BM) return PV_ERR_INVALID_ARG;
    if (a->epilogue != PV_EPI_BIAS_GELU_BF16 && a->epilogue != PV_EPI_BIAS_RES_F32) return PV_ERR_UNSUPPORTED;
    if (a->K % (2 * G2_BK) || a->N % 8) return PV_ERR_UNSUPPORTED;
    if (a->M > 0x7fffffff || a->N > 0x7fffffff || a->K > 0x7fffffff || tiles_m * ((a->N + G2_BN - 1) / G2_BN) > 0x7fffffff) return PV_ERR_UNSUPPORTED;
    if (a->lda % 8 || a->ldw % 8 || a->ldo % 8 || a->lda < a->K || a->ldw < a->K || a->ldo < a->N) return PV_ERR_INVALID_ARG;
    if (a->lda > (0x7fffffffLL - 56) / 255 || a->ldw > (0x7fffffffLL - 56) / 255 ||
        (a->epilogue == PV_EPI_BIAS_GELU_BF16 && a->ldo > (0x7fffffffLL - 248) / 255)) return PV_ERR_UNSUPPORTED;
    if (w_stride < a->N * a->ldw) return PV_ERR_INVALID_ARG;
    if (((uintptr_t)a->A & 15) || ((uintptr_t)a->W & 15) || ((uintptr_t)a->out & 15) || (a->bias && ((uintptr_t)a->bias & 15))) return PV_ERR_INVALID_ARG;
    if (a->bias && (a->N % 4)) return PV_ERR_INVALID_ARG;
    if ((uintptr_t)a->range_flag & 3) return PV_ERR_INVALID_ARG;
    if (a->row_scale || a->pos || a->ln_out || a->x16_out || a->rowstat_out || a->fold_stat || a->rowsq_out || a->colsum_partial || a->ksplit > 1 ||
        a->qcols || a->res_scaled) return PV_ERR_INVALID_ARG;
    if (a->epilogue == PV_EPI_BIAS_RES_F32 && (!a->res || !perm || out_rows <= 0 || out_rows > 0x7fffffff || a->ldr % 4 || a->ldr < a->N ||
                                               ((uintptr_t)a->res & 15) || ((uintptr_t)perm & 3))) return PV_ERR_INVALID_ARG;
    GemmDev p = {};
    p.A = a->A; p.W = a->W; p.bias = a->bias; p.out = a->out; p.res = a->res;
    p.M = (int)a->M; p.N = (int)a->N; p.K = (int)a->K;
    p.lda = a->lda; p.ldw = a->ldw; p.ldo = a->ldo; p.ldr = a->ldr;
    p.qscale = 1.0f; p.ksplit = 1; p.k_slice = p.K;
    p.range_flag = a->range_flag;
    p.row_map = perm; p.map_rows = (int)out_rows;
    p.tiles_m = (int)tiles_m; p.tiles_n = (p.N + G2_BN - 1) / G2_BN; p.gm = 1; p.gc = p.tiles_n;
#ifdef PV_STAMPS
    p.dbg = nullptr;
#endif
    PvGroupDev g;
    g.tile_expert = tile_expert; g.w_stride = w_stride; g.E = (int)E;
    hipStream_t s = (hipStream_t)stream;
    const dim3 grid((unsigned)(p.tiles_m * p.tiles_n));
    if (a->epilogue == PV_EPI_BIAS_GELU_BF16) {
        static PvPerDevice attr_set;
        constexpr int lds = G2_LDS + PV_GELU_CUB_N * PV_GELU_CUB_REP * 16 + 4096;
        if (attr_set.first_use())
            (void)hipFuncSetAttribute(reinterpret_cast<const void*>(static_cast<void (*)(const GemmDev, const PvGroupDev)>(pv_gemm256_kernel<PV_EPI_BIAS_GELU_BF16>)),
                                      hipFuncAttributeMaxDynamicSharedMemorySize, lds);
        PV_LAUNCH((static_cast<void (*)(const GemmDev, const PvGroupDev)>(pv_gemm256_kernel<PV_EPI_BIAS_GELU_BF16>)), grid, dim3(512), lds, s, p, g);
    } else {
        static PvPerDevice attr_set;
        constexpr int lds = G2_LDS;
        if (attr_set.first_use())
            (void)hipFuncSetAttribute(reinterpret_cast<const void*>(static_cast<void (*)(const GemmDev, const PvGroupDev)>(pv_gemm256_kernel<PV_EPI_BIAS_RES_F32>)),
                                      hipFuncAttributeMaxDynamicSharedMemorySize, lds);
        PV_LAUNCH((static_cast<void (*)(const GemmDev, const PvGroupDev)>(pv_gemm256_kernel<PV_EPI_BIAS_RES_F32>)), grid, dim3(512), lds, s, p, g);
    }
    return pv_check_launch();
}
```

### peekvit_amd/engine.py

```python
from __future__ import annotations

import math
import os
import threading
import warnings
import weakref
from typing import Dict, List, Optional, Tuple

import torch
from torch import nn

from . import _lib, autograph, ops
import contextlib

from ._lib import (PV_EPI_BIAS_BF16, PV_EPI_BIAS_F32, PV_EPI_BIAS_GELU_BF16, PV_EPI_BIAS_GELU_SPLIT_BF16, PV_EPI_BIAS_POS_F32,
                   PV_EPI_BIAS_RES_F32, PeekvitHipError)

_MODE_DEFAULT = os.environ.get("PEEKVIT_AMD_PRECISION", "auto")
_MODES = ("auto", "bf16", "f16", "bf16x3")
if _MODE_DEFAULT not in _MODES:
    raise ValueError(f"PEEKVIT_AMD_PRECISION={_MODE_DEFAULT!r}: expected one of {_MODES}")
_lib._OPERAND_DEFAULT = "f16" if _MODE_DEFAULT == "f16" else "bf16"
_mode_tls = threading.local()

# ... 633 lines not shown
            _wcache[key] = ent[:5] + (True,)
        return ent[3]
    src = p.detach()
    if src.dtype != torch.float32:
        src = src.float()
    if not src.is_contiguous():
        src = src.contiguous()
    with torch.inference_mode(False):
        w = ops.cast_bf16(src.view(src.shape[0], -1))
    checked = _lib.OPERAND != "f16"
    if _lib.OPERAND == "f16" and not getattr(_region, "no_param_checks", False):
        _check_f16_cast(src.view(src.shape[0], -1), w)
        checked = True
    ev = None
    if _STREAMS > 1 and not torch.cuda.is_current_stream_capturing():
        ev = (torch.cuda.current_stream(p.device).cuda_stream, torch.cuda.Event())
        ev[1].record()
    _wcache[key] = (weakref.ref(p, lambda _r, k=key: _wcache.pop(k, None)), pver(p), p.data_ptr(), w, ev, checked)
    return w


IMAGENET_MEAN, IMAGENET_STD = (0.485, 0.456, 0.406), (0.229, 0.224, 0.225)


_normcache: Dict[tuple, Tuple[torch.Tensor, torch.Tensor]] = {}


def norm_constants(model: nn.Module, device) -> Tuple[torch.Tensor, torch.Tensor]:
    mean, std = tuple(getattr(model, "input_mean", IMAGENET_MEAN)), tuple(getattr(model, "input_std", IMAGENET_STD))
    key = (torch.device(device), mean, std)
    ent = _normcache.get(key)
    if ent is None:
        with torch.inference_mode(False):
            ent = _normcache[key] = (torch.tensor(mean, dtype=torch.float32, device=device).view(1, -1, 1, 1),
                                     torch.tensor(std, dtype=torch.float32, device=device).view(1, -1, 1, 1))
    return ent


_w3cache: Dict[int, Tuple["weakref.ref", int, int, torch.Tensor]] = {}


def bf16x3_weight(p: torch.Tensor) -> torch.Tensor:
    key = id(p)
    ent = _w3cache.get(key)
    if ent is not None and ent[0]() is p and ent[1] == pver(p) and ent[2] == p.data_ptr():
        return ent[3]
    src = p.detach()
    src = (src if src.is_contiguous() else src.contiguous()).view(src.shape[0], -1)
    with torch.inference_mode(False):
        w = ops.split3(src, 1)
    _w3cache[key] = (weakref.ref(p, lambda _r, k=key: _w3cache.pop(k, None)), pver(p), p.data_ptr(), w)
    return w


def _f32(p: Optional[torch.Tensor]) -> Optional[torch.Tensor]:
    if p is None:
        return None
    d = p.detach()
    if d.dtype != torch.float32:
        d = d.float()
    return d if d.is_contiguous() else d.contiguous()


_FUSE_LN = os.environ.get("PEEKVIT_AMD_FUSE_LN", "0") == "1"


_FULLROW_LN = os.environ.get("PEEKVIT_AMD_FULLROW_LN", "1") == "1"


def _ln_fusable(D: int, K: int) -> bool:
    if _FULLROW_LN and D in (256, 384, 512) and K % 64 == 0:
        return True
    return _FUSE_LN and D % 256 == 0 and D <= 4096 and K % 128 == 0


def _ln_key(ln: nn.LayerNorm):
    return (id(ln.weight), pver(ln.weight), pver(ln.bias), float(ln.eps))


_FOLD_LN = os.environ.get("PEEKVIT_AMD_FOLD_LN", "1") == "1"
_foldok_cache: Dict[Tuple[int, int, int, str], bool] = {}
_FUSE_RANK_NORM = os.environ.get("PEEKVIT_AMD_FUSE_RANK_NORM", "1") == "1"
_foldcache: Dict[Tuple[int, int, str], tuple] = {}


def _fold_weights(w: torch.Tensor, b: Optional[torch.Tensor], ln: nn.LayerNorm):
    key = (id(w), id(ln.weight), _lib.OPERAND)
    ver = (pver(w), pver(b) if b is not None else -1, pver(ln.weight), pver(ln.bias), w.data_ptr())
    ent = _foldcache.get(key)
    if ent is not None and ent[0] == ver:
        return ent[1]
    with torch.inference_mode(False), torch.no_grad():
        wf = w.detach().float()
        wsrc = (wf * ln.weight.detach().float()).contiguous()
        wg = ops.cast_bf16(wsrc)
        if _lib.OPERAND == "f16":
            _check_f16_cast(wsrc, wg)
        c1 = wg.float().sum(1).contiguous()
        c2 = (wf @ ln.bias.detach().float() + (b.detach().float() if b is not None else 0.0)).contiguous()
    if key not in _foldcache:
        _evict_with(w, _foldcache, key)
        _evict_with(ln.weight, _foldcache, key)
    _foldcache[key] = (ver, (wg, c1, c2))
    return wg, c1, c2


def _fold_ok(R: int, D: int, M: int) -> bool:
    if not (_FOLD_LN and _mode() in ("bf16", "f16") and D % 128 == 0 and M % 128 == 0) or _ln_fusable(D, D):
        return False
    if getattr(_region, "no_fold", False):
        return False
    key = (R, D, M, _lib.OPERAND)
    ok = _foldok_cache.get(key)
    if ok is None:
        ok = _foldok_cache[key] = all(ops.gemm_tile_rows(R, n, k, epi) == 256 for n, k, epi in (
            (3 * D, D, PV_EPI_BIAS_BF16), (D, D, PV_EPI_BIAS_RES_F32), (M, D, PV_EPI_BIAS_GELU_BF16), (D, M, PV_EPI_BIAS_RES_F32)))
    return ok


_SMALL_M_SPLITK = os.environ.get("PEEKVIT_AMD_SPLITK", "1") != "0"


def _splitk_slices(M: int, N: int, K: int, min_k: int = 2048) -> int:
    if not _SMALL_M_SPLITK or K < min_k:
        return 1
    tiles = ((M + 127) // 128) * ((N + 127) // 128)
    if tiles >= 256:
        return 1
    best = 1
    for s_ in (2, 3, 4, 6, 8, 12, 16):
        if K % (s_ * 64) == 0 and K // s_ >= 256 and tiles * s_ <= 768:
            best = s_
    return best


def _residual_gemm(a: torch.Tensor, w: torch.Tensor, bias: torch.Tensor, out2d: torch.Tensor, res2d: torch.Tensor, M: int, ln=None) -> bool:
    N, K = w.shape[0], a.shape[-1]
    ks = _splitk_slices(M, N, K, 512 if ln is not None else 1024) if res2d.is_contiguous() and out2d.is_contiguous() else 1
    if ks > 1:
        part = workspace.get("splitk", (ks, M, N), torch.float32, a.device)
        ops.gemm(a, w, bias, part, PV_EPI_BIAS_F32, M=M, ksplit=ks)
        ops.sum_slices(part, out2d, base=res2d, ln=ln)
        return ln is not None
    ops.gemm(a, w, bias, out2d, PV_EPI_BIAS_RES_F32, M=M, res=res2d)
    return False


def _act_gemm(a: torch.Tensor, w: torch.Tensor, bias: torch.Tensor, out: torch.Tensor, M: int, gelu: bool, qcols: int = 0, qscale: float = 1.0):
    N, K = w.shape[0], a.shape[-1]
    ks = _splitk_slices(M, N, K, 512) if gelu and out.is_contiguous() else 1
    if ks > 1:
        part = workspace.get("splitk", (ks, M, N), torch.float32, a.device)
        ops.gemm(a, w, bias, part, PV_EPI_BIAS_F32, M=M, ksplit=ks)
        return ops.sum_slices_act(part, out, gelu=gelu, qcols=qcols, qscale=qscale)
    return ops.gemm(a, w, bias, out, PV_EPI_BIAS_GELU_BF16 if gelu else PV_EPI_BIAS_BF16, M=M, qcols=qcols, qscale=qscale)


def _attention_half_split(blk: nn.Module, x: torch.Tensor, att: torch.Tensor, B: int, S: int, eps: float, row_scale: Optional[torch.Tensor]):
    mha = blk.self_attention.self_attention
    D = x.shape[-1]
    H = mha.num_heads
    dh = D // H
    R, dev = B * S, x.device
    old = _lib.set_operand("bf16")
    try:
        h3 = workspace.get("h3", (R, 3 * D), torch.bfloat16, dev)
        qkv32 = workspace.get("qkv32", (R, 3 * D), torch.float32, dev)
        ops.layernorm_split(x, _f32(blk.ln_1.weight), _f32(blk.ln_1.bias), eps, h3, row_scale)
        ops.gemm(h3, bf16x3_weight(mha.in_proj_weight), _f32(mha.in_proj_bias), qkv32, PV_EPI_BIAS_F32, M=R, qcols=D, qscale=float(dh) ** -0.5)
    finally:
        _lib.set_operand(old)
    ops.attention_split(qkv32, att, B, S, H, dh)


def _mlp_half_split(blk: nn.Module, x1: torch.Tensor, out: torch.Tensor, R: int, eps: float, row_scale: Optional[torch.Tensor]):
    D, M = x1.shape[-1], blk.mlp.fc1.out_features
    dev = x1.device
    old = _lib.set_operand("bf16")
    try:
        h3 = workspace.get("h3", (R, 3 * D), torch.bfloat16, dev)
        g3 = workspace.get("g3", (R, 3 * M), torch.bfloat16, dev)
        ops.layernorm_split(x1, _f32(blk.ln_2.weight), _f32(blk.ln_2.bias), eps, h3, row_scale)
        ops.gemm(h3, bf16x3_weight(blk.mlp.fc1.weight), _f32(blk.mlp.fc1.bias), g3, PV_EPI_BIAS_GELU_SPLIT_BF16, M=R)
        ops.gemm(g3, bf16x3_weight(blk.mlp.fc2.weight), _f32(blk.mlp.fc2.bias), out.view(R, D), PV_EPI_BIAS_RES_F32, M=R, res=x1.view(R, D))
    finally:
        _lib.set_operand(old)


def block_forward(blk: nn.Module, x: torch.Tensor, eps: float, row_scale: Optional[torch.Tensor] = None,
                  next_ln: Optional[nn.LayerNorm] = None, next_ranks: bool = False, h1: Optional[torch.Tensor] = None,
                  res_scaled: bool = False) -> torch.Tensor:
    if _mode() == "bf16x3":
        return _block_forward_x3(blk, x, eps, row_scale)
    if x.dtype != torch.float32:
        x = x.float()
    handoff = getattr(x, "_pv_ln", None)
    if not x.is_contiguous():
        x, handoff = x.contiguous(), None
    B, S, D = x.shape
    mha = blk.self_attention.self_attention
    H = mha.num_heads
    dh = D // H
    M = blk.mlp.fc1.out_features
    dev = x.device
    R = B * S

    _check_ln_range(blk.ln_1)
    _check_ln_range(blk.ln_2)
    h2 = workspace.get("h2", (R, D), _lib.operand_dtype(), dev)
    qkv = workspace.get("qkv", (R, 3 * D), _lib.operand_dtype(), dev)
    att = workspace.get("att", (R, D), _lib.operand_dtype(), dev)
    g = workspace.get("g", (R, M), _lib.operand_dtype(), dev)
    x1 = workspace.get("x1", (B, S, D), torch.float32, dev)
    out = torch.empty_like(x)

    hyb = layer_is_hybrid()
    if row_scale is None and _fold_ok(R, D, M):
        nt = (D + 255) // 256
        fold_in = getattr(x, "_pv_fold", None)
        if fold_in is not None and fold_in[3] != _tver(x):
            fold_in = None
        if hyb:
            _attention_half_split(blk, x, att, B, S, eps, None)
        elif fold_in is not None and fold_in[2] == _ln_key(blk.ln_1) and fold_in[0].shape == (R, D):
            wg, c1, c2 = _fold_weights(mha.in_proj_weight, mha.in_proj_bias, blk.ln_1)
            stat = ops.rowstat_finalize(fold_in[1], D, blk.ln_1.eps, workspace.get("fold_stat", (R, 2), torch.float32, dev))
            ops.gemm(fold_in[0], wg, None, qkv, PV_EPI_BIAS_BF16, M=R, qcols=D, qscale=float(dh) ** -0.5, fold=(stat, c1, c2))
        else:
            h = workspace.get("h", (R, D), _lib.operand_dtype(), dev)
            ops.layernorm_bf16(x, _f32(blk.ln_1.weight), _f32(blk.ln_1.bias), eps, h, None)
            ops.gemm(h, bf16_weight(mha.in_proj_weight), _f32(mha.in_proj_bias), qkv, PV_EPI_BIAS_BF16, M=R, qcols=D, qscale=float(dh) ** -0.5)
        if not hyb:
            ops.attention(qkv, att, B, S, H, dh)
        x16 = workspace.get("fold_x16", (R, D), _lib.operand_dtype(), dev)
        part = workspace.get("fold_part", (nt, R, 2), torch.float32, dev)
        mlp_hyb = layer_mlp_is_hybrid()
        ops.gemm(att, bf16_weight(mha.out_proj.weight), _f32(mha.out_proj.bias), x1.view(R, D), PV_EPI_BIAS_RES_F32, M=R, res=x.view(R, D),
                 x16_out=None if mlp_hyb else x16, rowstat_out=None if mlp_hyb else part)
        if mlp_hyb:
            _mlp_half_split(blk, x1, out, R, eps, None)
            return out
        wg, c1, c2 = _fold_weights(blk.mlp.fc1.weight, blk.mlp.fc1.bias, blk.ln_2)
        stat = ops.rowstat_finalize(part, D, blk.ln_2.eps, workspace.get("fold_stat", (R, 2), torch.float32, dev))
        ops.gemm(x16, wg, None, g, PV_EPI_BIAS_GELU_BF16, M=R, fold=(stat, c1, c2))
        emit = next_ln is not None and next_ln.normalized_shape == (D,)
        o16 = workspace.get("fold_o16", (R, D), _lib.operand_dtype(), dev) if emit else None
        opart = workspace.get("fold_opart", (nt, R, 2), torch.float32, dev) if emit else None
        rowsq = workspace.get("rowsq", (nt, R), torch.float32, dev) if (next_ranks and not emit and _FUSE_RANK_NORM) else None
        ops.gemm(g, bf16_weight(blk.mlp.fc2.weight), _f32(blk.mlp.fc2.bias), out.view(R, D), PV_EPI_BIAS_RES_F32, M=R, res=x1.view(R, D),
                 x16_out=o16, rowstat_out=opart, rowsq_out=rowsq)
        if emit:
            out._pv_fold = (o16, opart, _ln_key(next_ln), _tver(out))
        if rowsq is not None:
            out._pv_rowsq = (rowsq, _tver(out))
        return out

    if hyb:
        if res_scaled:
            raise PeekvitHipError("block_forward(res_scaled=True) cannot run a hybrid layer: pass the masked tokens")
        _attention_half_split(blk, x, att, B, S, eps, row_scale)
    else:
        if h1 is not None and h1.shape == (R, D):
            h = h1
        elif handoff is not None and row_scale is None and handoff[1] == _ln_key(blk.ln_1) and handoff[0].shape == (R, D):
            h = handoff[0]
        else:
            h = workspace.get("h", (R, D), _lib.operand_dtype(), dev)
            ops.layernorm_bf16(x, _f32(blk.ln_1.weight), _f32(blk.ln_1.bias), eps, h, row_scale)
        ops.gemm(h, bf16_weight(mha.in_proj_weight), _f32(mha.in_proj_bias), qkv, PV_EPI_BIAS_BF16, M=R,
                 qcols=D, qscale=float(dh) ** -0.5)
        ops.attention(qkv, att, B, S, H, dh)
    mlp_hyb = layer_mlp_is_hybrid()
    if mlp_hyb and res_scaled:
        raise PeekvitHipError("block_forward(res_scaled=True) cannot run a layer whose MLP half is in split precision: pass the masked tokens")
    fuse2 = _ln_fusable(D, D) and not mlp_hyb
    if res_scaled and (h1 is None or row_scale is None or fuse2):
        raise PeekvitHipError("block_forward(res_scaled=True) needs row_scale, the caller's h1 and the tile GEMM (no full-row LayerNorm fusion)")
    if fuse2 or row_scale is not None:
        ops.gemm(att, bf16_weight(mha.out_proj.weight), _f32(mha.out_proj.bias), x1.view(R, D), PV_EPI_BIAS_RES_F32, M=R,
                 res=x.view(R, D), row_scale=row_scale, res_scaled=res_scaled,
                 ln=(_f32(blk.ln_2.weight), _f32(blk.ln_2.bias), eps, h2, row_scale) if fuse2 else None)
        ln2_done = fuse2
    else:
        ln2_done = _residual_gemm(att, bf16_weight(mha.out_proj.weight), _f32(mha.out_proj.bias), x1.view(R, D), x.view(R, D), R,
                                  ln=(_f32(blk.ln_2.weight), _f32(blk.ln_2.bias), eps, h2))
    if mlp_hyb:
        _mlp_half_split(blk, x1, out, R, eps, row_scale)
        return out
    if not ln2_done:
        ops.layernorm_bf16(x1, _f32(blk.ln_2.weight), _f32(blk.ln_2.bias), eps, h2, row_scale)
    _act_gemm(h2, bf16_weight(blk.mlp.fc1.weight), _f32(blk.mlp.fc1.bias), g, R, gelu=True)
    fuse_next = next_ln is not None and _ln_fusable(D, M) and next_ln.normalized_shape == (D,)
    hn = workspace.get("h", (R, D), _lib.operand_dtype(), dev) if fuse_next else None
    rowsq = None
    if next_ranks and not fuse_next and _FUSE_RANK_NORM and ops.gemm_tile_rows(R, D, M, PV_EPI_BIAS_RES_F32) == 256:
        rowsq = workspace.get("rowsq", ((D + 255) // 256, R), torch.float32, dev)
    if fuse_next or rowsq is not None:
        ops.gemm(g, bf16_weight(blk.mlp.fc2.weight), _f32(blk.mlp.fc2.bias), out.view(R, D), PV_EPI_BIAS_RES_F32, M=R,
                 res=x1.view(R, D), rowsq_out=rowsq,
                 ln=(_f32(next_ln.weight), _f32(next_ln.bias), next_ln.eps, hn, None) if fuse_next else None)
    else:
        want = next_ln is not None and next_ln.normalized_shape == (D,)
        hn = workspace.get("h", (R, D), _lib.operand_dtype(), dev) if want else None
        fuse_next = _residual_gemm(g, bf16_weight(blk.mlp.fc2.weight), _f32(blk.mlp.fc2.bias), out.view(R, D), x1.view(R, D), R,
                                   ln=(_f32(next_ln.weight), _f32(next_ln.bias), next_ln.eps, hn) if want else None)
    if fuse_next:
        out._pv_ln = (hn, _ln_key(next_ln))
    if rowsq is not None:
        out._pv_rowsq = (rowsq, _tver(out))
    return out


_LAST_BLOCK_ROWS = os.environ.get("PEEKVIT_AMD_LAST_BLOCK_ROWS", "1") != "0"
_GATE_LN1 = os.environ.get("PEEKVIT_AMD_GATE_LN1", "1") != "0"
_GATE_NO_MASKED = os.environ.get("PEEKVIT_AMD_GATE_MASKED", "0") != "1"


def rows_only_ok(blk: nn.Module) -> bool:
    import torch.nn.modules.module as _m
    if not _LAST_BLOCK_ROWS or _mode() == "bf16x3" or layer_is_hybrid() or layer_mlp_is_hybrid():
        return False
    own = ("_forward_hooks", "_forward_pre_hooks", "_backward_hooks", "_backward_pre_hooks")
    glob = ("_global_forward_hooks", "_global_forward_pre_hooks", "_global_backward_hooks", "_global_backward_pre_hooks")
    return not any(getattr(blk, n, None) for n in own) and not any(getattr(_m, n, None) for n in glob)


def block_forward_rows(blk: nn.Module, x: torch.Tensor, eps: float, nq: int, row_scale: Optional[torch.Tensor] = None,
                       h1: Optional[torch.Tensor] = None) -> torch.Tensor:
    if x.dtype != torch.float32:
        x = x.float()
    fold_in, handoff = getattr(x, "_pv_fold", None), getattr(x, "_pv_ln", None)
    if fold_in is not None and fold_in[3] != _tver(x):
        fold_in = None
# ... 951 lines not shown
```

### peekvit_amd/ops.py

```python
from __future__ import annotations

import ctypes as C
from typing import Optional

import torch

from . import _lib
from ._lib import GemmArgs, check

launch_count = 0


class KernelTimer:

    def __init__(self):
        self.records = []

    def __enter__(self):
        global _timer
        _timer = self
        return self

    def __exit__(self, *exc):
        global _timer
# ... 133 lines not shown
    _, S, D = tokens.shape
    if H != W or w.shape != (D, Cc * patch * patch) or pos.shape[1] != D or pos.shape[0] < row_off + (H // patch) ** 2:
        raise _lib.PeekvitHipError(f"patch_embed: shapes x {tuple(x.shape)}, w {tuple(w.shape)}, pos {tuple(pos.shape)}, tokens {tuple(tokens.shape)}")
    M = B * (H // patch) ** 2
    with _timed("pv_gemm_bf16", x.device, 2.0 * M * D * w.shape[1], 4.0 * x.numel() + 2.0 * w.numel() + 4.0 * M * D, member=(D, w.shape[1], _lib.PV_EPI_BIAS_POS_F32)):
        check(_lib.load().pv_patch_embed_f32(_ptr(x), _ptr(w), _ptr(bias), _ptr(pos), _ptr(tokens), B, Cc, H, patch, D, S, row_off, _flag(x.device), _stream(x)),
              "pv_patch_embed_f32")
    _count()
    return tokens


def im2col(x: torch.Tensor, patch: int, out: torch.Tensor) -> torch.Tensor:
    _chk(x, torch.float32, "x")
    B, Cc, H, W = x.shape
    with _timed("pv_im2col_bf16", x.device, 0.0, 6.0 * x.numel()):
        check(_lib.load().pv_im2col_bf16(_ptr(x), _ptr(out), B, Cc, H, W, patch, _flag(x.device), _stream(x)), "pv_im2col_bf16")
    _count()
    return out


def im2col_u8(x: torch.Tensor, patch: int, out: torch.Tensor, mean, std) -> torch.Tensor:
    _chk(x, torch.uint8, "x")
    B, H, W, Cc = x.shape
    if Cc != 3:
        raise _lib.PeekvitHipError("uint8 input must be NHWC with 3 channels")
    with _timed("pv_im2col_u8_bf16", x.device, 0.0, 3.0 * x.numel()):
        check(_lib.load().pv_im2col_u8_bf16(_ptr(x), _ptr(out), B, H, W, patch, *[float(v) for v in mean], *[float(v) for v in std],
                                            _stream(x)), "pv_im2col_u8_bf16")
    _count()
    return out


def token_prologue(tokens, special, pos, budget_token, budget: float, n_special: int):
    B, S, D = tokens.shape
    with _timed("pv_token_prologue", tokens.device, 0.0, 0.0):
        check(_lib.load().pv_token_prologue(_ptr(tokens), _ptr(special), _ptr(pos), _ptr(budget_token), float(budget),
                                            B, S, D, n_special, _stream(tokens)), "pv_token_prologue")
    _count()


def layernorm_bf16(x: torch.Tensor, gamma, beta, eps: float, out: torch.Tensor, row_scale=None):
    D = x.shape[-1]
    rows = x.numel() // D
    with _timed("pv_layernorm_bf16", x.device, 0.0, 6.0 * x.numel()):
        check(_lib.load().pv_layernorm_bf16(_ptr(x), D, _ptr(gamma), _ptr(beta), _ptr(row_scale), _ptr(out), rows, D,
                                            float(eps), _stream(x)), "pv_layernorm_bf16")
    _count()
    return out


def gemm(a: torch.Tensor, w: torch.Tensor, bias, out: torch.Tensor, epilogue: int, *, M=None, res=None,
         row_scale=None, pos=None, rows_per_img_in=0, rows_per_img_out=0, row_off=0, qcols=0, qscale=1.0, ln=None, ksplit=0, tag="", colsum_out=None, x16_out=None, rowstat_out=None, fold=None, rowsq_out=None, res_scaled=False):
    K = a.shape[-1]
    if M is None:
        M = a.numel() // K
    N = w.shape[0]
    range_flag = current_range_flag()
    args = GemmArgs(A=a.data_ptr(), W=w.data_ptr(), bias=bias.data_ptr() if bias is not None else 0,
                    out=out.data_ptr(), res=res.data_ptr() if res is not None else 0,
                    row_scale=row_scale.data_ptr() if row_scale is not None else 0,
                    pos=pos.data_ptr() if pos is not None else 0,
                    M=M, N=N, K=K, lda=a.stride(0) if a.dim() == 2 else K, ldw=w.stride(0) if w.dim() == 2 else w.shape[-1],
                    ldo=out.stride(-2) if out.dim() >= 2 else out.shape[-1],
                    ldr=(res.stride(0) if res.dim() == 2 else res.shape[-1]) if res is not None else 0,
                    rows_per_img_in=rows_per_img_in, rows_per_img_out=rows_per_img_out, row_off=row_off,
                    qcols=qcols, qscale=float(qscale), epilogue=epilogue,
                    ln_gamma=ln[0].data_ptr() if ln else 0, ln_beta=ln[1].data_ptr() if ln else 0,
                    ln_row_scale=ln[4].data_ptr() if ln and ln[4] is not None else 0,
                    ln_out=ln[3].data_ptr() if ln else 0, ln_eps=float(ln[2]) if ln else 0.0, ksplit=int(ksplit), colsum_partial=0,
                    x16_out=x16_out.data_ptr() if x16_out is not None else 0, rowstat_out=rowstat_out.data_ptr() if rowstat_out is not None else 0,
                    fold_stat=fold[0].data_ptr() if fold else 0, fold_c1=fold[1].data_ptr() if fold else 0, fold_c2=fold[2].data_ptr() if fold else 0,
                    range_flag=range_flag.data_ptr() if range_flag is not None and range_flag.device == a.device else 0,
                    rowsq_out=rowsq_out.data_ptr() if rowsq_out is not None else 0, res_scaled=int(res_scaled))
    part = None
    if colsum_out is not None and _lib.load().pv_gemm_tile_rows(C.byref(args)) == 256:
        part = _scratch_f32(_lib.PV_WS_GEMM_COLSUM_PARTIAL, a.device, M, N).view((M + 255) // 256, N)
        args.colsum_partial = part.data_ptr()
    nbytes = 2.0 * (M * K + N * K) + out.element_size() * M * N * (2 if res is not None else 1) + (2.0 * M * N if ln else 0.0) + (2.0 * M * N if x16_out is not None else 0.0)
    with _timed("pv_gemm_bf16" + tag, a.device, 2.0 * M * N * K, nbytes, member=(N, K, epilogue)):
        check(_lib.load().pv_gemm_bf16(C.byref(args), _stream(a)), "pv_gemm_bf16")
    _count()
    if colsum_out is not None:
        colsum(part if part is not None else out, colsum_out)
    return out


def rowstat_finalize(partials: torch.Tensor, D: int, eps: float, out: Optional[torch.Tensor] = None) -> torch.Tensor:
    _chk(partials, torch.float32, "partials")
    T, rows, _ = partials.shape
    if out is None:
        out = torch.empty((rows, 2), dtype=torch.float32, device=partials.device)
    with _timed("pv_rowstat_finalize", partials.device, 0.0, 8.0 * (T + 1) * rows):
        check(_lib.load().pv_rowstat_finalize(_ptr(partials), _ptr(out), T, rows, D, float(eps), _flag(partials.device), _stream(partials)), "pv_rowstat_finalize")
    _count()
    return out


def gemm_tn(a: torch.Tensor, b: torch.Tensor, part: torch.Tensor, ksplit: int, tag: str = "[wgrad]"):
    K, M = a.shape
    N = b.shape[1]
    ldo = part.stride(1)
    assert b.shape[0] == K and part.shape == (max(ksplit, 1), M, N) and part.stride(2) == 1 and ldo >= N and part.stride(0) == M * ldo
    args = GemmArgs(A=a.data_ptr(), W=b.data_ptr(), bias=0, out=part.data_ptr(), res=0, row_scale=0, pos=0, M=M, N=N, K=K,
                    lda=a.stride(0), ldw=b.stride(0), ldo=ldo, ldr=0, rows_per_img_in=0, rows_per_img_out=0, row_off=0, qcols=0,
                    qscale=1.0, epilogue=_lib.PV_EPI_BIAS_F32, ln_gamma=0, ln_beta=0, ln_row_scale=0, ln_out=0, ln_eps=0.0,
                    ksplit=int(ksplit))
    with _timed("pv_gemm_tn_bf16" + tag, a.device, 2.0 * M * N * K, 2.0 * K * (M + N) + 4.0 * max(ksplit, 1) * M * N):
        check(_lib.load().pv_gemm_tn_bf16(C.byref(args), _stream(a)), "pv_gemm_tn_bf16")
    _count()
    return part


def attention(qkv: torch.Tensor, out: torch.Tensor, B: int, S: int, H: int, dh: int, lse: Optional[torch.Tensor] = None):
    with _timed("pv_attention_bf16", qkv.device, 4.0 * B * H * S * S * dh, 8.0 * B * S * H * dh):
        if lse is None:
            check(_lib.load().pv_attention_bf16(_ptr(qkv), _ptr(out), B, S, H, dh, _attn_flag(qkv.device), _stream(qkv)), "pv_attention_bf16")
        else:
            _chk(lse, torch.float32, "lse")
            if lse.numel() != B * H * S:
                raise _lib.PeekvitHipError("attention: lse must hold B * H * S values")
            check(_lib.load().pv_attention_lse_bf16(_ptr(qkv), _ptr(out), _ptr(lse), B, S, H, dh, _attn_flag(qkv.device), _stream(qkv)), "pv_attention_lse_bf16")
    _count()
    return out


def attention_bwd_lse_ok(S: int, dh: int) -> bool:
    return attention_bwd_lse_supported(S, dh) and S >= 145


def attention_bwd_lse_supported(S: int, dh: int) -> bool:
    return dh in (48, 64) and 129 <= S <= 208


def attention_rows(q: torch.Tensor, kv: torch.Tensor, out: torch.Tensor, B: int, S: int, nq: int, H: int, dh: int):
    for t, name in ((q, "q"), (kv, "kv"), (out, "out")):
        if not (t.is_cuda and t.dtype == _lib.operand_dtype() and t.dim() == 2 and t.stride(1) == 1):
            raise _lib.PeekvitHipError(f"attention_rows: {name} must be a 2-D GPU tensor of the operand type with unit column stride")
    if q.shape[0] != B * nq or out.shape[0] != B * nq or kv.shape[0] != B * S or kv.shape[1] < 2 * H * dh:
        raise _lib.PeekvitHipError("attention_rows: shape mismatch")
    with _timed("pv_attention_rows_bf16", q.device, 4.0 * B * H * nq * S * dh, 4.0 * B * S * H * dh + 4.0 * B * nq * H * dh):
        check(_lib.load().pv_attention_rows_bf16(_ptr(q), q.stride(0), _ptr(kv), kv.stride(0), _ptr(out), out.stride(0),
                                                 B, S, nq, H, dh, _attn_flag(q.device), _stream(q)), "pv_attention_rows_bf16")
    _count()
    return out


def attention_rows_bwd(q, kv, out, dout, dq, dkv, B: int, S: int, H: int, dh: int, qscale: float):
    for t, name in ((q, "q"), (kv, "kv"), (out, "out"), (dout, "dout"), (dq, "dq"), (dkv, "dkv")):
        if not (t.is_cuda and t.dtype == _lib.operand_dtype() and t.dim() == 2 and t.stride(1) == 1):
            raise _lib.PeekvitHipError(f"attention_rows_bwd: {name} must be a 2-D GPU tensor of the operand type with unit column stride")
    if any(t.shape[0] != B for t in (q, out, dout, dq)) or kv.shape[0] != B * S or dkv.shape[0] != B * S:
        raise _lib.PeekvitHipError("attention_rows_bwd: shape mismatch")
    with _timed("pv_attention_rows_bwd_bf16", q.device, 10.0 * B * H * S * dh, 2.0 * 3 * 2 * B * S * H * dh):
        check(_lib.load().pv_attention_rows_bwd_bf16(_ptr(q), q.stride(0), _ptr(kv), kv.stride(0), _ptr(out), out.stride(0), _ptr(dout), dout.stride(0),
                                                     _ptr(dq), dq.stride(0), _ptr(dkv), dkv.stride(0), B, S, 1, H, dh, float(qscale), _stream(q)),
              "pv_attention_rows_bwd_bf16")
    _count()
    return dq, dkv


def cls_pool(x: torch.Tensor, gamma, beta, eps: float, num_cls: int) -> torch.Tensor:
    B, S, D = x.shape
    pooled = torch.empty((B, D), dtype=torch.float32, device=x.device)
    with _timed("pv_cls_pool", x.device, 0.0, 0.0):
        check(_lib.load().pv_cls_pool(_ptr(x), _ptr(gamma), _ptr(beta), _ptr(pooled), B, S, D, num_cls, float(eps),
                                      _stream(x)), "pv_cls_pool")
# ... 1522 lines not shown
```

Before: 28010 images/sec.

## Store mid-block residual as operand hi plane plus 8-bit remainder plane

Between the attention out-proj GEMM and the fc2 GEMM, the fp32 residual x1 is no longer written and reread. It is stored as the 16-bit operand copy (already produced for the next GEMM) plus an 8-bit remainder plane in a tiled layout. fc2 then reconstructs an approximate fp32 residual from the two planes. This cuts residual traffic from 4+4 bytes to about 1+1 extra bytes per element, but the residual is only approximately fp32 (16-bit value plus 8 more mantissa bits), and it adds new epilogue kernels and a fixed tile-layout constraint.

```diff
diff --git a/include/peekvit_hip_res8.h b/include/peekvit_hip_res8.h
--- /dev/null
+++ b/include/peekvit_hip_res8.h
@@ -0,0 +1,28 @@
+#ifndef PEEKVIT_HIP_RES8_H
+#define PEEKVIT_HIP_RES8_H
+
+#include "peekvit_hip.h"
+
+#ifdef __cplusplus
+extern "C" {
+#endif
+
+typedef struct pv_res8_args {
+    uint64_t struct_size;
+    const uint16_t* res_hi;
+    const uint8_t* res_lo;
+    uint16_t* out_hi;
+    uint8_t* out_lo;
+    int64_t lo_rows;
+} pv_res8_args;
+
+int pv_gemm_res8_bf16(const pv_gemm_args* a, const pv_res8_args* r, void* stream);
+
+int pv_res8_decode_f32(const uint16_t* hi, const uint8_t* lo, float* out, int64_t M, int64_t N, int64_t lo_rows, void* stream);
+
+int pv_res8_tile_ok(const pv_gemm_args* a);
+
+#ifdef __cplusplus
+}
+#endif
+#endif
diff --git a/peekvit_amd/_build.py b/peekvit_amd/_build.py
--- a/peekvit_amd/_build.py
+++ b/peekvit_amd/_build.py
@@ -14,7 +14,7 @@
 HEADERS = ("peekvit_hip.h", "peekvit_hip_moe.h", "peekvit_hip_ee.h", "peekvit_hip_sparse.h", "peekvit_hip_pct.h",
            "peekvit_hip_pct_train.h", "peekvit_hip_attn_stream.h", "peekvit_hip_pct_block.h", "peekvit_hip_rank_train.h", "peekvit_hip_rank_infer.h",
            "peekvit_hip_avit_train.h", "peekvit_hip_sparse_train.h", "peekvit_hip_avit_pack_train.h", "peekvit_hip_dropout.h", "peekvit_hip_sparse_long.h",
-           "peekvit_hip_sparse_long_train.h", "peekvit_hip_avit_long.h")
+           "peekvit_hip_sparse_long_train.h", "peekvit_hip_avit_long.h", "peekvit_hip_res8.h")
 FILE_FLAGS = {"pv_attention.hip": ["-mllvm", "-amdgpu-mfma-vgpr-form=1"], "pv_rowops.hip": ["-fno-slp-vectorize"],
               "pv_attention_stream.hip": ["-mllvm", "-amdgpu-mfma-vgpr-form=1"],
               "pv_ee.hip": ["-fno-slp-vectorize"],
diff --git a/peekvit_amd/_lib.py b/peekvit_amd/_lib.py
--- a/peekvit_amd/_lib.py
+++ b/peekvit_amd/_lib.py
@@ -192,6 +192,22 @@
     "pv_avit_pack_step_long_bwd": SIGNATURES_AVIT_PACK_TRAIN["pv_avit_pack_step_bwd"],
 }
 
+
+
+class Res8Args(C.Structure):
+    _fields_ = [("struct_size", C.c_uint64), ("res_hi", _p), ("res_lo", _p), ("out_hi", _p), ("out_lo", _p), ("lo_rows", _i64)]
+
+    def __init__(self, *args, **kw):
+        super().__init__(*args, **kw)
+        self.struct_size = C.sizeof(Res8Args)
+
+
+SIGNATURES_RES8 = {
+    "pv_gemm_res8_bf16": (C.c_int, [C.POINTER(GemmArgs), C.POINTER(Res8Args), _p]),
+    "pv_res8_decode_f32": (C.c_int, [_p, _p, _p, _i64, _i64, _i64, _p]),
+    "pv_res8_tile_ok": (C.c_int, [C.POINTER(GemmArgs)]),
+}
+
 ABI_VERSION = 10
 _lock = threading.Lock()
 _libs: dict = {}
@@ -249,7 +265,7 @@
                                    **SIGNATURES_PCT_TRAIN, **SIGNATURES_ATTN_STREAM, **SIGNATURES_PCT_BLOCK, **SIGNATURES_RANK_TRAIN,
                                    **SIGNATURES_RANK_INFER, **SIGNATURES_AVIT_TRAIN, **SIGNATURES_SPARSE_TRAIN, **SIGNATURES_AVIT_PACK_TRAIN,
                                    **SIGNATURES_DROPOUT, **SIGNATURES_SPARSE_LONG, **SIGNATURES_SPARSE_LONG_TRAIN,
-                                   **SIGNATURES_AVIT_LONG}.items():
+                                   **SIGNATURES_AVIT_LONG, **SIGNATURES_RES8}.items():
             fn = getattr(lib, name)
             fn.restype, fn.argtypes = res, args
         if lib.pv_version() != ABI_VERSION:
diff --git a/peekvit_amd/csrc/pv_gemm.hip b/peekvit_amd/csrc/pv_gemm.hip
--- a/peekvit_amd/csrc/pv_gemm.hip
+++ b/peekvit_amd/csrc/pv_gemm.hip
@@ -1,5 +1,6 @@
 #include "pv_rows.h"
 #include "../../include/peekvit_hip_moe.h"
+#include "../../include/peekvit_hip_res8.h"
 #include "pv_gelu_table.h"
 #include <type_traits>
 #include <cstdlib>
@@ -127,7 +128,7 @@
     const uint16_t* W;
     const float* bias;
     void* out;
-    const float* res;
+    union { const float* res; const uint16_t* r8_hi; };
     const float* row_scale;
     const float* pos;
     int M, N, K;
@@ -143,7 +144,7 @@
     float* rowsq_out;
     int res_scaled;
     int k_last;
-    float* colsum_partial;
+    union { float* colsum_partial; uint8_t* r8_lo_out; };
     uint16_t* x16_out;
     float* rowstat_out;
     const float* fold_stat;
@@ -157,12 +158,28 @@
     const float* ln_row_scale;
     uint16_t* ln_out;
     float ln_eps;
-    const int* row_map;
+    union { const int* row_map; const uint8_t* r8_lo; };
     int map_rows;
 #ifdef PV_STAMPS
     unsigned long long* dbg;
 #endif
 };
+
+constexpr int PV_RES8_SH = PV_OPERAND_CODE ? 5 : 8;
+__device__ __forceinline__ float pv_res8_decode(float hi, uint32_t lo_word, int byte) {
+    const int q = __builtin_amdgcn_sbfe((int)lo_word, 8 * byte, 8);
+    return __builtin_bit_cast(float, (int)__builtin_bit_cast(uint32_t, hi) + (q << PV_RES8_SH) + (1 << (PV_RES8_SH - 1)));
+}
+__device__ __forceinline__ uint32_t pv_res8_encode(float x, float hi) {
+    int d = ((int)__builtin_bit_cast(uint32_t, x) - (int)__builtin_bit_cast(uint32_t, hi)) >> PV_RES8_SH;
+    d = d < -128 ? -128 : (d > 127 ? 127 : d);
+    return (uint32_t)d & 0xffu;
+}
+__host__ __device__ __forceinline__ int64_t pv_res8_lo_offset(int64_t m, int64_t n, int64_t N) {
+    const int64_t tile = (m >> 8) * (N >> 8) + (n >> 8);
+    const int r = (int)(m & 255), c = (int)(n & 255), j = r & 7;
+    return tile * 65536 + (r >> 6) * 16384 + ((r >> 3) & 7) * 2048 + (j >> 2) * 1024 + ((j & 1) * 32 + (c >> 3)) * 16 + ((j >> 1) & 1) * 8 + (c & 7);
+}
 
 #ifdef PV_STAMPS
 static unsigned long long* g_pv_dbg = nullptr;
@@ -543,7 +560,7 @@
 constexpr int G2_BUF = 4 * G2_HALF;
 constexpr int G2_LDS = 2 * G2_BUF;
 
-template <int EPI, bool PF = false, bool FULL = false, bool PERM = false>
+template <int EPI, bool PF = false, bool FULL = false, bool PERM = false, int R8 = 0>
 __device__ __forceinline__ void pv_gemm256_tile(const GemmDev& p, char* smem, const int m0, const int n0, const bool first = true,
                                                 const bool has_next = false, const int nm0 = 0, const int nn0 = 0, const int wid_pf = 0, const int slot_pf = 0) {
     int tid_ = threadIdx.x;
@@ -1045,6 +1062,133 @@
             }
         }
         if (!SPLIT) pv_range_commit(vmax, p.range_flag);
+    } else if constexpr (R8 != 0) {
+        constexpr bool R8_IN = (R8 & 1) != 0, R8_OUT = (R8 & 2) != 0;
+        float vmax = 0.f;
+        lds_c* const img = cimg + G2_BUF;
+        const int l31 = lane & 31, hrow = lane >> 5;
+        const int col = n0 + 8 * l31;
+        const int64_t lo_base = ((int64_t)(m0 / G2_BM) * (p.N / G2_BN) + n0 / G2_BN) * 65536 + wid * 2048 + lane * 16;
+        u32x4 rh[2][R8_IN ? 4 : 8];
+        u32x4 rl[2][R8_IN ? 2 : 1];
+        auto fetch = [&](int q) __attribute__((always_inline)) {
+#pragma unroll
+            for (int jj = 0; jj < 4; ++jj) {
+                int m = m0 + q * 64 + wid * 8 + 2 * jj + hrow;
+                m = (FULL || m < p.M) ? m : p.M - 1;
+                if constexpr (R8_IN) {
+                    rh[q & 1][jj] = *reinterpret_cast<const u32x4*>(p.r8_hi + (int64_t)m * p.ldr + col);
+                } else {
+                    rh[q & 1][2 * jj] = *reinterpret_cast<const u32x4*>(p.res + (int64_t)m * p.ldr + col);
+                    rh[q & 1][2 * jj + 1] = *reinterpret_cast<const u32x4*>(p.res + (int64_t)m * p.ldr + col + 4);
+                }
+            }
+            if constexpr (R8_IN) {
+#pragma unroll
+                for (int pp = 0; pp < 2; ++pp) rl[q & 1][pp] = *reinterpret_cast<const u32x4*>(p.r8_lo + lo_base + q * 16384 + pp * 1024);
+            }
+        };
+        fetch(0);
+        fetch(1);
+        if (PFM == 2 && pf_next) {
+#pragma unroll
+            for (int pc = 0; pc < 9; ++pc) stage_next_piece(nm0, nn0, pc);
+        }
+#pragma unroll
+        for (int q = 0; q < 4; ++q) {
+            if (q > 0) __builtin_amdgcn_s_barrier();
+            if (wr == (q >> 1)) {
+#pragma unroll
+                for (int ml = 0; ml < 4; ++ml) {
+                    const int mt = 4 * (q & 1) + ml, row = ml * 16 + i16;
+#pragma unroll
+                    for (int nt = 0; nt < 4; ++nt) {
+                        const int c = wc * 16 + (nt >> 1) * 8 + g * 2 + (nt & 1);
+                        *reinterpret_cast<__attribute__((address_space(3))) f32x4*>(img + row * 1024 + ((c ^ (i16 & 7)) << 4)) = acc[nt][mt];
+                    }
+                }
+            }
+            asm volatile("s_waitcnt lgkmcnt(0)" ::: "memory");
+            __builtin_amdgcn_s_barrier();
+            if (PFM == 1 && q == 0 && pf_next) asm volatile("s_waitcnt vmcnt(0)" ::: "memory");
+            float fs[2][4], fq[2][4];
+            u32x4 lo_out[2];
+#pragma unroll
+            for (int jj = 0; jj < 4; ++jj) {
+                const int row = wid * 8 + 2 * jj + hrow, c0 = 2 * l31;
+                const f32x4 va = *reinterpret_cast<const __attribute__((address_space(3))) f32x4*>(img + row * 1024 + ((c0 ^ (row & 7)) << 4));
+                const f32x4 vb = *reinterpret_cast<const __attribute__((address_space(3))) f32x4*>(img + row * 1024 + (((c0 + 1) ^ (row & 7)) << 4));
+                float o[8];
+                if constexpr (R8_IN) {
+                    const u32x4 hd = rh[q & 1][jj];
+                    const u32x4 ld = rl[q & 1][jj >> 1];
+#pragma unroll
+                    for (int e = 0; e < 8; ++e) {
+                        const float h_ = (e & 1) ? pv_unpack_hi(hd[e >> 1]) : pv_unpack_lo(hd[e >> 1]);
+                        o[e] = pv_res8_decode(h_, ld[2 * (jj & 1) + (e >> 2)], e & 3);
+                    }
+                } else {
+#pragma unroll
+                    for (int e = 0; e < 8; ++e) o[e] = __builtin_bit_cast(float, rh[q & 1][2 * jj + (e >> 2)][e & 3]);
+                }
+#pragma unroll
+                for (int e = 0; e < 4; ++e) { o[e] = pv_add_s(va[e], o[e]); o[4 + e] = pv_add_s(vb[e], o[4 + e]); }
+                const u32x4 pk = {pv_pack_bf16x2_tracked(o[0], o[1], vmax), pv_pack_bf16x2_tracked(o[2], o[3], vmax),
+                                  pv_pack_bf16x2_tracked(o[4], o[5], vmax), pv_pack_bf16x2_tracked(o[6], o[7], vmax)};
+                const int mrow = m0 + q * 64 + row;
+                const bool ok = FULL || mrow < p.M;
+                if (ok) PV_STORE16(reinterpret_cast<u32x4*>(p.x16_out + (int64_t)mrow * p.N + col), pk);
+                if constexpr (R8_OUT) {
+                    uint32_t w[2];
+#pragma unroll
+                    for (int k = 0; k < 2; ++k) {
+                        w[k] = 0;
+#pragma unroll
+                        for (int b = 0; b < 4; ++b) {
+                            const int e = 4 * k + b;
+                            const float h_ = (e & 1) ? pv_unpack_hi(pk[e >> 1]) : pv_unpack_lo(pk[e >> 1]);
+                            w[k] |= pv_res8_encode(o[e], h_) << (8 * b);
+                        }
+                    }
+                    lo_out[jj >> 1][2 * (jj & 1)] = w[0]; lo_out[jj >> 1][2 * (jj & 1) + 1] = w[1];
+                    if (jj & 1) PV_STORE16(reinterpret_cast<u32x4*>(p.r8_lo_out + lo_base + q * 16384 + (jj >> 1) * 1024), lo_out[jj >> 1]);
+                } else if (ok) {
+                    float* const orow = reinterpret_cast<float*>(p.out) + (int64_t)mrow * p.ldo + col;
+                    PV_STORE32(reinterpret_cast<f32x4*>(orow), ((f32x4){o[0], o[1], o[2], o[3]}));
+                    PV_STORE32(reinterpret_cast<f32x4*>(orow + 4), ((f32x4){o[4], o[5], o[6], o[7]}));
+                }
+#pragma unroll
+                for (int k = 0; k < 2; ++k) {
+                    const float* const ok_ = o + 4 * k;
+                    fs[k][jj] = ok ? pv_add_s(pv_add_s(ok_[0], ok_[1]), pv_add_s(ok_[2], ok_[3])) : 0.f;
+                    fq[k][jj] = ok ? pv_add_s(pv_add_s(pv_mul_s(ok_[0], ok_[0]), pv_mul_s(ok_[1], ok_[1])), pv_add_s(pv_mul_s(ok_[2], ok_[2]), pv_mul_s(ok_[3], ok_[3]))) : 0.f;
+                }
+            }
+            if (q + 2 < 4) fetch(q + 2);
+            {
+                const bool b4 = lane & 16, b3 = lane & 8;
+                float tot[2][2];
+#pragma unroll
+                for (int k = 0; k < 2; ++k)
+#pragma unroll
+                    for (int s_ = 0; s_ < 2; ++s_) {
+                        const float(&v)[4] = s_ ? fq[k] : fs[k];
+                        float t2[2];
+#pragma unroll
+                        for (int i = 0; i < 2; ++i) t2[i] = pv_add_s(b4 ? v[i + 2] : v[i], __shfl_xor(b4 ? v[i] : v[i + 2], 16, 64));
+                        float t1 = pv_add_s(b3 ? t2[1] : t2[0], __shfl_xor(b3 ? t2[0] : t2[1], 8, 64));
+                        t1 = pv_add_s(t1, __shfl_xor(t1, 4, 64));
+                        t1 = pv_add_s(t1, __shfl_xor(t1, 2, 64));
+                        t1 = pv_add_s(t1, __shfl_xor(t1, 1, 64));
+                        tot[s_][k] = t1;
+                    }
+                const int mrow = m0 + q * 64 + wid * 8 + 2 * (2 * (int)b4 + (int)b3) + hrow;
+                if ((lane & 7) == 0 && mrow < p.M)
+                    *reinterpret_cast<float2*>(p.rowstat_out + ((int64_t)(n0 / G2_BN) * p.M + mrow) * 2) =
+                        make_float2(pv_add_s(tot[0][0], tot[0][1]), pv_add_s(tot[1][0], tot[1][1]));
+            }
+        }
+        pv_range_commit(vmax, p.range_flag);
     } else {
         constexpr bool DG = EPI == PV_EPI_GELU_GRAD_BF16;
         float cs8[DG ? 8 : 1];
@@ -1213,7 +1357,7 @@
         const bool full = FULL || (m0 + G2_BM <= p.M && n0 + G2_BN <= p.N);
         constexpr bool B16 = EPI == PV_EPI_BIAS_BF16 || EPI == PV_EPI_BIAS_GELU_BF16 || EPI == PV_EPI_BIAS_GELU_PAIR_BF16 || EPI == PV_EPI_GELU_GRAD_BF16;
         if (!full) asm volatile("s_waitcnt vmcnt(0)" ::: "memory");
-        else if (B16) asm volatile("s_waitcnt vmcnt(16)" ::: "memory");
+        else if (B16 || R8 != 0) asm volatile("s_waitcnt vmcnt(16)" ::: "memory");
         else asm volatile("s_waitcnt vmcnt(32)" ::: "memory");
     }
     PV_STAMP(3);
@@ -1230,9 +1374,8 @@
 #endif
 }
 
-template <int EPI>
-__global__ __launch_bounds__(512) void pv_gemm256_kernel(const GemmDev p_in) {
-    extern __shared__ __attribute__((aligned(16))) char smem[];
+template <int EPI, int R8>
+__device__ __forceinline__ void pv_gemm256_one_tile_body(const GemmDev& p_in, char* smem) {
     GemmDev p = p_in;
     const int ntiles = p.tiles_m * p.tiles_n;
     const int slice = blockIdx.x / ntiles;
@@ -1250,13 +1393,18 @@
     const int gsz = min(p.gm, p.tiles_m - grp * p.gm);
     const int tnl = rem / gsz, tm = grp * p.gm + (rem - tnl * gsz);
     const int m0 = tm * G2_BM, n0 = (ch * p.gc + tnl) * G2_BN;
-    if (m0 + G2_BM <= p.M && n0 + G2_BN <= p.N) pv_gemm256_tile<EPI, false, true>(p, smem, m0, n0);
-    else pv_gemm256_tile<EPI, false, false>(p, smem, m0, n0);
+    if (m0 + G2_BM <= p.M && n0 + G2_BN <= p.N) pv_gemm256_tile<EPI, false, true, false, R8>(p, smem, m0, n0);
+    else pv_gemm256_tile<EPI, false, false, false, R8>(p, smem, m0, n0);
 }
 
 template <int EPI>
-__global__ __launch_bounds__(512) void pv_gemm256_pf_kernel(const GemmDev p) {
+__global__ __launch_bounds__(512) void pv_gemm256_kernel(const GemmDev p_in) {
     extern __shared__ __attribute__((aligned(16))) char smem[];
+    pv_gemm256_one_tile_body<EPI, 0>(p_in, smem);
+}
+
+template <int EPI, int R8>
+__device__ __forceinline__ void pv_gemm256_pf_body(const GemmDev p, char* smem) {
     const int ntiles = p.tiles_m * p.tiles_n;
     const int xcd = blockIdx.x & 7, j = blockIdx.x >> 3, per = gridDim.x >> 3;
     const int q8 = ntiles >> 3, r8 = ntiles & 7;
@@ -1278,13 +1426,28 @@
     for (int i = j; i < cnt; i += per) {
         const bool has_next = i + per < cnt;
         if (has_next) decode(start + i + per, nm0, nn0);
-        if (m0 + G2_BM <= p.M && n0 + G2_BN <= p.N) pv_gemm256_tile<EPI, true, true>(p, smem, m0, n0, i == j, has_next, nm0, nn0, wid, start + i);
-        else pv_gemm256_tile<EPI, true, false>(p, smem, m0, n0, i == j, has_next, nm0, nn0, wid, start + i);
+        if (m0 + G2_BM <= p.M && n0 + G2_BN <= p.N) pv_gemm256_tile<EPI, true, true, false, R8>(p, smem, m0, n0, i == j, has_next, nm0, nn0, wid, start + i);
+        else pv_gemm256_tile<EPI, true, false, false, R8>(p, smem, m0, n0, i == j, has_next, nm0, nn0, wid, start + i);
         asm volatile("s_waitcnt lgkmcnt(0)" ::: "memory");
         __builtin_amdgcn_s_barrier();
         __builtin_amdgcn_sched_barrier(0);
         m0 = nm0; n0 = nn0;
     }
+}
+template <int EPI>
+__global__ __launch_bounds__(512) void pv_gemm256_pf_kernel(const GemmDev p) {
+    extern __shared__ __attribute__((aligned(16))) char smem[];
+    pv_gemm256_pf_body<EPI, 0>(p, smem);
+}
+template <int R8>
+__global__ __launch_bounds__(512) void pv_gemm256_res8_kernel(const GemmDev p) {
+    extern __shared__ __attribute__((aligned(16))) char smem[];
+    pv_gemm256_one_tile_body<PV_EPI_BIAS_RES_F32, R8>(p, smem);
+}
+template <int R8>
+__global__ __launch_bounds__(512) void pv_gemm256_res8_pf_kernel(const GemmDev p) {
+    extern __shared__ __attribute__((aligned(16))) char smem[];
+    pv_gemm256_pf_body<PV_EPI_BIAS_RES_F32, R8>(p, smem);
 }
 
 struct PvGroupDev {
@@ -1630,6 +1793,23 @@
     return pv_check_launch();
 }
 
+template <int R8>
+static int pv_launch_gemm256_res8(const GemmDev& p, hipStream_t stream) {
+    static PvPerDevice attr_set;
+    constexpr int lds = G2_LDS, lds_pf = G2_LDS + 4096 + 1024;
+    if (attr_set.first_use()) {
+        (void)hipFuncSetAttribute(reinterpret_cast<const void*>(pv_gemm256_res8_kernel<R8>), hipFuncAttributeMaxDynamicSharedMemorySize, lds);
+        (void)hipFuncSetAttribute(reinterpret_cast<const void*>(pv_gemm256_res8_pf_kernel<R8>), hipFuncAttributeMaxDynamicSharedMemorySize, lds_pf);
+    }
+    const int cus = pv_cu_count();
+    if (pv_gemm_pf_enabled() && p.K >= 4 * G2_BK && (int64_t)p.tiles_m * p.tiles_n >= 2 * (int64_t)cus && cus >= 8) {
+        PV_LAUNCH(pv_gemm256_res8_pf_kernel<R8>, dim3((unsigned)(cus & ~7)), dim3(512), lds_pf, stream, p);
+        return pv_check_launch();
+    }
+    PV_LAUNCH(pv_gemm256_res8_kernel<R8>, dim3((unsigned)(p.tiles_m * p.tiles_n)), dim3(512), lds, stream, p);
+    return pv_check_launch();
+}
+
 template <int EPI>
 static int pv_launch_gemm256_rows(const GemmDev& p, hipStream_t stream) {
     static PvPerDevice attr_set;
@@ -2085,7 +2265,7 @@
 static int g_pv_fullrow = -1;
 extern "C" void pv_debug_set_gemm_fullrow(int on) { g_pv_fullrow = on; }
 
-static int pv_gemm_dispatch(const pv_gemm_args* a, void* stream, bool query_only);
+static int pv_gemm_dispatch(const pv_gemm_args* a, void* stream, bool query_only, const pv_res8_args* r8 = nullptr);
 extern "C" int pv_gemm_bf16(const pv_gemm_args* a, void* stream) { return pv_gemm_dispatch(a, stream, false); }
 extern "C" int pv_gemm_tile_rows(const pv_gemm_args* a) {
     if (!a || a->struct_size != sizeof(pv_gemm_args)) return PV_ERR_INVALID_ARG;
@@ -2093,7 +2273,7 @@
     q.colsum_partial = nullptr; q.x16_out = nullptr; q.rowstat_out = nullptr; q.fold_stat = nullptr; q.rowsq_out = nullptr;
     return pv_gemm_dispatch(&q, nullptr, true);
 }
-static int pv_gemm_dispatch(const pv_gemm_args* a, void* stream, bool query_only) {
+static int pv_gemm_dispatch(const pv_gemm_args* a, void* stream, bool query_only, const pv_res8_args* r8) {
     if (!a || a->struct_size != sizeof(pv_gemm_args)) return PV_ERR_INVALID_ARG;
     if (!a->A || !a->W || !a->out || a->M <= 0 || a->N <= 0 || a->K <= 0) return PV_ERR_INVALID_ARG;
     if (a->K % 64 || a->N % 4) return PV_ERR_UNSUPPORTED;
@@ -2160,6 +2340,7 @@
     const bool fullrow_shape = a->epilogue == PV_EPI_BIAS_RES_F32 && (p.N == 256 || p.N == 384 || p.N == 512) && p.ksplit <= 1 && !feat &&
                                (g_pv_fullrow >= 0 ? g_pv_fullrow != 0 : fullrow_env != 0) && force == 0;
     if (a->ln_out && !fullrow_shape && !ld_ok256) return PV_ERR_UNSUPPORTED;
+    if (r8 && !big) return PV_ERR_UNSUPPORTED;
     if (query_only) return big ? G2_BM : G1_BM;
     if ((a->epilogue == PV_EPI_BIAS_BF16 || a->epilogue == PV_EPI_BIAS_F32) && p.qcols % 4) return PV_ERR_UNSUPPORTED;
     static const int gm_env = [] { const char* e = getenv("PV_GEMM_GM"); return e ? atoi(e) : 0; }();
@@ -2181,6 +2362,12 @@
         p.tiles_m = (p.M + G2_BM - 1) / G2_BM; p.tiles_n = p.N / G2_BN;
         return pv_launch_gemm256_rows<PV_EPI_BIAS_RES_F32>(p, s);
     }
+    if (r8) {
+        if (r8->res_hi) { p.r8_hi = r8->res_hi; p.r8_lo = r8->res_lo; }
+        if (r8->out_hi) p.r8_lo_out = r8->out_lo;
+        const int mode = (r8->res_hi ? 1 : 0) | (r8->out_hi ? 2 : 0);
+        return mode == 1 ? pv_launch_gemm256_res8<1>(p, s) : mode == 2 ? pv_launch_gemm256_res8<2>(p, s) : pv_launch_gemm256_res8<3>(p, s);
+    }
     switch (a->epilogue) {
         case PV_EPI_BIAS_BF16: return big ? pv_launch_gemm256<PV_EPI_BIAS_BF16>(p, s) : pv_launch_gemm128<PV_EPI_BIAS_BF16>(p, s);
         case PV_EPI_BIAS_GELU_BF16: return big ? pv_launch_gemm256<PV_EPI_BIAS_GELU_BF16>(p, s) : pv_launch_gemm128<PV_EPI_BIAS_GELU_BF16>(p, s);
@@ -2196,6 +2383,66 @@
         case PV_EPI_GELU_GRAD_BF16: return big ? pv_launch_gemm256<PV_EPI_GELU_GRAD_BF16>(p, s) : pv_launch_gemm128<PV_EPI_GELU_GRAD_BF16>(p, s);
         default: return PV_ERR_INVALID_ARG;
     }
+}
+
+static bool pv_res8_plain(const pv_gemm_args* a) {
+    return a->epilogue == PV_EPI_BIAS_RES_F32 && a->N % G2_BN == 0 && !a->row_scale && !a->res_scaled && !a->ln_out && a->ksplit <= 1 && !a->rowsq_out &&
+           !a->pos && !a->colsum_partial && !a->fold_stat;
+}
+
+extern "C" int pv_res8_tile_ok(const pv_gemm_args* a) {
+    if (!a || a->struct_size != sizeof(pv_gemm_args)) return PV_ERR_INVALID_ARG;
+    if (!pv_res8_plain(a)) return 0;
+    pv_gemm_args q = *a;
+    q.res = reinterpret_cast<const float*>(uintptr_t(16)); q.out = reinterpret_cast<void*>(uintptr_t(16));
+    q.x16_out = reinterpret_cast<uint16_t*>(uintptr_t(16)); q.rowstat_out = reinterpret_cast<float*>(uintptr_t(16));
+    const pv_res8_args r = {};
+    return pv_gemm_dispatch(&q, nullptr, true, &r) == G2_BM ? 1 : 0;
+}
+
+extern "C" int pv_gemm_res8_bf16(const pv_gemm_args* a, const pv_res8_args* r, void* stream) {
+    if (!a || a->struct_size != sizeof(pv_gemm_args) || !r || r->struct_size != sizeof(pv_res8_args)) return PV_ERR_INVALID_ARG;
+    if ((r->res_hi != nullptr) != (r->res_lo != nullptr) || (r->out_hi != nullptr) != (r->out_lo != nullptr)) return PV_ERR_INVALID_ARG;
+    if (!r->res_hi && !r->out_hi) return PV_ERR_INVALID_ARG;
+    if (r->out_hi ? (a->out || a->x16_out) : (!a->out || !a->x16_out)) return PV_ERR_INVALID_ARG;
+    if (r->res_hi ? a->res != nullptr : !a->res) return PV_ERR_INVALID_ARG;
+    if (!a->rowstat_out || a->M <= 0 || a->N <= 0) return PV_ERR_INVALID_ARG;
+    if (((uintptr_t)r->res_hi & 15) || ((uintptr_t)r->res_lo & 15) || ((uintptr_t)r->out_hi & 15) || ((uintptr_t)r->out_lo & 15) ||
+        ((uintptr_t)a->x16_out & 15)) return PV_ERR_INVALID_ARG;
+    if (r->lo_rows % G2_BM || r->lo_rows < (a->M + G2_BM - 1) / G2_BM * G2_BM) return PV_ERR_INVALID_ARG;
+    if (r->res_hi && (r->res_hi == r->out_hi || r->res_lo == r->out_lo || (const void*)r->res_hi == (const void*)a->x16_out)) return PV_ERR_INVALID_ARG;
+    if (r->res_hi && (a->ldr % 8 || a->ldr < a->N)) return PV_ERR_INVALID_ARG;
+    if (!pv_res8_plain(a)) return PV_ERR_UNSUPPORTED;
+    pv_gemm_args q = *a;
+    if (r->res_hi) q.res = reinterpret_cast<const float*>(r->res_hi);
+    if (r->out_hi) { q.out = r->out_hi; q.x16_out = r->out_hi; q.ldo = a->N; }
+    return pv_gemm_dispatch(&q, stream, false, r);
+}
+
+__global__ __launch_bounds__(256) void pv_res8_decode_kernel(const uint16_t* __restrict__ hi, const uint8_t* __restrict__ lo, float* __restrict__ out,
+                                                             int64_t chunks, int N) {
+    for (int64_t i = (int64_t)blockIdx.x * 256 + threadIdx.x; i < chunks; i += (int64_t)gridDim.x * 256) {
+        const int64_t m = i / (N >> 3);
+        const int n = (int)(i - m * (N >> 3)) << 3;
+        const u32x4 h = *reinterpret_cast<const u32x4*>(hi + m * N + n);
+        const u32x2 l = *reinterpret_cast<const u32x2*>(lo + pv_res8_lo_offset(m, n, N));
+        f32x4 o[2];
+#pragma unroll
+        for (int e = 0; e < 8; ++e)
+            o[e >> 2][e & 3] = pv_res8_decode((e & 1) ? pv_unpack_hi(h[e >> 1]) : pv_unpack_lo(h[e >> 1]), l[e >> 2], e & 3);
+        *reinterpret_cast<f32x4*>(out + m * N + n) = o[0];
+        *reinterpret_cast<f32x4*>(out + m * N + n + 4) = o[1];
+    }
+}
+
+extern "C" int pv_res8_decode_f32(const uint16_t* hi, const uint8_t* lo, float* out, int64_t M, int64_t N, int64_t lo_rows, void* stream) {
+    if (!hi || !lo || !out || M <= 0 || N <= 0) return PV_ERR_INVALID_ARG;
+    if (((uintptr_t)hi & 15) || ((uintptr_t)lo & 15) || ((uintptr_t)out & 15)) return PV_ERR_INVALID_ARG;
+    if (lo_rows % G2_BM || lo_rows < (M + G2_BM - 1) / G2_BM * G2_BM) return PV_ERR_INVALID_ARG;
+    if (N % G2_BN || N > 0x7fffffff || M > 0x7fffffff) return PV_ERR_UNSUPPORTED;
+    const int64_t chunks = M * (N >> 3);
+    PV_LAUNCH(pv_res8_decode_kernel, dim3(pv_stream_grid(chunks, 256)), dim3(256), 0, (hipStream_t)stream, hi, lo, out, chunks, (int)N);
+    return pv_check_launch();
 }
 
 extern "C" int pv_gemm_grouped_bf16(const pv_gemm_args* a, const int32_t* tile_expert, int64_t tiles_m, int64_t E, int64_t w_stride,
diff --git a/peekvit_amd/engine.py b/peekvit_amd/engine.py
--- a/peekvit_amd/engine.py
+++ b/peekvit_amd/engine.py
@@ -739,6 +739,16 @@
 _foldok_cache: Dict[Tuple[int, int, int, str], bool] = {}
 _FUSE_RANK_NORM = os.environ.get("PEEKVIT_AMD_FUSE_RANK_NORM", "1") == "1"
 _foldcache: Dict[Tuple[int, int, str], tuple] = {}
+_RES8 = os.environ.get("PEEKVIT_AMD_RES8", "1") != "0"
+_res8ok_cache: Dict[Tuple[int, int, int, str], bool] = {}
+
+
+def _res8_ok(R: int, D: int, M: int) -> bool:
+    key = (R, D, M, _lib.OPERAND)
+    ok = _res8ok_cache.get(key)
+    if ok is None:
+        ok = _res8ok_cache[key] = ops.res8_tile_ok(R, D, D) and ops.res8_tile_ok(R, D, M)
+    return ok
 
 
 def _fold_weights(w: torch.Tensor, b: Optional[torch.Tensor], ln: nn.LayerNorm):
@@ -892,20 +902,29 @@
         x16 = workspace.get("fold_x16", (R, D), _lib.operand_dtype(), dev)
         part = workspace.get("fold_part", (nt, R, 2), torch.float32, dev)
         mlp_hyb = layer_mlp_is_hybrid()
-        ops.gemm(att, bf16_weight(mha.out_proj.weight), _f32(mha.out_proj.bias), x1.view(R, D), PV_EPI_BIAS_RES_F32, M=R, res=x.view(R, D),
-                 x16_out=None if mlp_hyb else x16, rowstat_out=None if mlp_hyb else part)
+        emit = next_ln is not None and next_ln.normalized_shape == (D,)
+        want_rowsq = next_ranks and not emit and _FUSE_RANK_NORM
+        x1_lo = None
+        if _RES8 and not mlp_hyb and not want_rowsq and _res8_ok(R, D, M):
+            x1_lo = workspace.get("x1_lo", (ops.res8_lo_rows(R) * D,), torch.uint8, dev)
+            ops.gemm_res8(att, bf16_weight(mha.out_proj.weight), _f32(mha.out_proj.bias), M=R, rowstat_out=part, res=x.view(R, D), out8=(x16, x1_lo))
+        else:
+            ops.gemm(att, bf16_weight(mha.out_proj.weight), _f32(mha.out_proj.bias), x1.view(R, D), PV_EPI_BIAS_RES_F32, M=R, res=x.view(R, D),
+                     x16_out=None if mlp_hyb else x16, rowstat_out=None if mlp_hyb else part)
         if mlp_hyb:
             _mlp_half_split(blk, x1, out, R, eps, None)
             return out
         wg, c1, c2 = _fold_weights(blk.mlp.fc1.weight, blk.mlp.fc1.bias, blk.ln_2)
         stat = ops.rowstat_finalize(part, D, blk.ln_2.eps, workspace.get("fold_stat", (R, 2), torch.float32, dev))
         ops.gemm(x16, wg, None, g, PV_EPI_BIAS_GELU_BF16, M=R, fold=(stat, c1, c2))
-        emit = next_ln is not None and next_ln.normalized_shape == (D,)
-        o16 = workspace.get("fold_o16", (R, D), _lib.operand_dtype(), dev) if emit else None
-        opart = workspace.get("fold_opart", (nt, R, 2), torch.float32, dev) if emit else None
-        rowsq = workspace.get("rowsq", (nt, R), torch.float32, dev) if (next_ranks and not emit and _FUSE_RANK_NORM) else None
-        ops.gemm(g, bf16_weight(blk.mlp.fc2.weight), _f32(blk.mlp.fc2.bias), out.view(R, D), PV_EPI_BIAS_RES_F32, M=R, res=x1.view(R, D),
-                 x16_out=o16, rowstat_out=opart, rowsq_out=rowsq)
+        o16 = workspace.get("fold_o16", (R, D), _lib.operand_dtype(), dev) if emit or x1_lo is not None else None
+        opart = workspace.get("fold_opart", (nt, R, 2), torch.float32, dev) if emit or x1_lo is not None else None
+        rowsq = workspace.get("rowsq", (nt, R), torch.float32, dev) if want_rowsq else None
+        if x1_lo is not None:
+            ops.gemm_res8(g, bf16_weight(blk.mlp.fc2.weight), _f32(blk.mlp.fc2.bias), M=R, rowstat_out=opart, res8=(x16, x1_lo), out=out.view(R, D), x16_out=o16)
+        else:
+            ops.gemm(g, bf16_weight(blk.mlp.fc2.weight), _f32(blk.mlp.fc2.bias), out.view(R, D), PV_EPI_BIAS_RES_F32, M=R, res=x1.view(R, D),
+                     x16_out=o16, rowstat_out=opart, rowsq_out=rowsq)
         if emit:
             out._pv_fold = (o16, opart, _ln_key(next_ln), _tver(out))
         if rowsq is not None:
diff --git a/peekvit_amd/ops.py b/peekvit_amd/ops.py
--- a/peekvit_amd/ops.py
+++ b/peekvit_amd/ops.py
@@ -239,6 +239,56 @@
     _count()
     if colsum_out is not None:
         colsum(part if part is not None else out, colsum_out)
+    return out
+
+
+def res8_lo_rows(M: int) -> int:
+    return (M + 255) // 256 * 256
+
+
+def res8_tile_ok(M: int, N: int, K: int, **fields) -> bool:
+    args = GemmArgs(A=16, W=16, out=16, res=16, M=M, N=N, K=K, lda=K, ldw=K, ldo=N, ldr=N, qscale=1.0, epilogue=_lib.PV_EPI_BIAS_RES_F32)
+    for name, value in fields.items():
+        setattr(args, name, value)
+    return int(_lib.load().pv_res8_tile_ok(C.byref(args))) == 1
+
+
+def gemm_res8(a: torch.Tensor, w: torch.Tensor, bias, *, M: int, rowstat_out: torch.Tensor, res=None, res8=None, out=None, x16_out=None, out8=None):
+    K, N = a.shape[-1], w.shape[0]
+    if (res is None) == (res8 is None) or (out8 is None) == (out is None) or (out8 is None) != (x16_out is not None) or (res8 is None and out8 is None):
+        raise _lib.PeekvitHipError("gemm_res8: give res or res8, and out + x16_out or out8, with a plane pair on at least one side")
+    lo_rows = res8_lo_rows(M)
+    for pair in (res8, out8):
+        if pair is not None:
+            _chk(pair[0], _lib.operand_dtype(), "hi"); _chk(pair[1], torch.uint8, "lo")
+            if pair[0].numel() < M * N or pair[1].numel() < lo_rows * N:
+                raise _lib.PeekvitHipError(f"gemm_res8: planes hold {pair[0].numel()} values and {pair[1].numel()} remainders, need {M * N} and {lo_rows * N}")
+    range_flag = current_range_flag()
+    args = GemmArgs(A=a.data_ptr(), W=w.data_ptr(), bias=bias.data_ptr() if bias is not None else 0, out=out.data_ptr() if out is not None else 0,
+                    res=res.data_ptr() if res is not None else 0, M=M, N=N, K=K, lda=a.stride(0) if a.dim() == 2 else K,
+                    ldw=w.stride(0) if w.dim() == 2 else w.shape[-1], ldo=(out.stride(-2) if out.dim() >= 2 else N) if out is not None else N,
+                    ldr=(res.stride(0) if res.dim() == 2 else N) if res is not None else N, qscale=1.0, epilogue=_lib.PV_EPI_BIAS_RES_F32,
+                    x16_out=x16_out.data_ptr() if x16_out is not None else 0, rowstat_out=rowstat_out.data_ptr(),
+                    range_flag=range_flag.data_ptr() if range_flag is not None and range_flag.device == a.device else 0)
+    r = _lib.Res8Args(res_hi=res8[0].data_ptr() if res8 else 0, res_lo=res8[1].data_ptr() if res8 else 0,
+                      out_hi=out8[0].data_ptr() if out8 else 0, out_lo=out8[1].data_ptr() if out8 else 0, lo_rows=lo_rows)
+    nbytes = 2.0 * (M * K + N * K) + float(M * N) * ((3 if res8 else 4) + (3 if out8 else 6))
+    with _timed("pv_gemm_bf16", a.device, 2.0 * M * N * K, nbytes, member=(N, K, _lib.PV_EPI_BIAS_RES_F32)):
+        check(_lib.load().pv_gemm_res8_bf16(C.byref(args), C.byref(r), _stream(a)), "pv_gemm_res8_bf16")
+    _count()
+    return out if out8 is None else out8
+
+
+def res8_decode(hi: torch.Tensor, lo: torch.Tensor, out: torch.Tensor, M: Optional[int] = None) -> torch.Tensor:
+    _chk(hi, _lib.operand_dtype(), "hi"); _chk(lo, torch.uint8, "lo"); _chk(out, torch.float32, "out")
+    N = hi.shape[-1]
+    if M is None:
+        M = hi.numel() // N
+    if out.numel() < M * N or lo.numel() < res8_lo_rows(M) * N:
+        raise _lib.PeekvitHipError("res8_decode: out or lo is too small for the rows of hi")
+    with _timed("pv_res8_decode_f32", hi.device, 0.0, 7.0 * M * N):
+        check(_lib.load().pv_res8_decode_f32(_ptr(hi), _ptr(lo), _ptr(out), M, N, res8_lo_rows(M), _stream(hi)), "pv_res8_decode_f32")
+    _count()
     return out
 
 
```

Result: slower. 13490 images/sec (-51.8%).
